# arielgabizon/barretenberg

Hardware: AMD Instinct MI355X
Metric: BN254 G1 MSM points/sec at n=2^20 (Fr NTT elems/sec in 'ntt') (higher is better)
Workload: dtype u32x9 (256-bit Montgomery, 29-bit limbs)

## Files before the change

### barretenberg_amd/csrc/msm.hip

```cpp
#include <hip/hip_runtime.h>

#include <algorithm>
#include <mutex>
#include <stdint.h>
#include <stdio.h>
#include <stdlib.h>
#include <string.h>
#include <vector>

#include "bbgpu_internal.h"
#include "g1.hpp"
#include "g1_quad.hpp"
#include "host_g1.hpp"

namespace bbgpu {

using Fr = FrP;
#ifndef BBGPU_FRONT_PRIO
#define BBGPU_FRONT_PRIO 2
#endif
#define FRONT_PRIO() __builtin_amdgcn_s_setprio(BBGPU_FRONT_PRIO)
#ifndef BBGPU_TAIL_PRIO
#define BBGPU_TAIL_PRIO 3
#endif
constexpr int SCALAR_BITS = 254;
constexpr int MSM_MAX_C = 16;
constexpr int MSM_THREADS = 256;

__device__ __forceinline__ void ld8(const uint32_t* p, uint32_t (&w)[8])
{
    const uint4* q = reinterpret_cast<const uint4*>(p);
    uint4 a = q[0], b = q[1];
    w[0] = a.x; w[1] = a.y; w[2] = a.z; w[3] = a.w;
    w[4] = b.x; w[5] = b.y; w[6] = b.z; w[7] = b.w;
}
__device__ __forceinline__ void ld16(const uint32_t* p, uint32_t (&w)[16])
{
    const uint4* q = reinterpret_cast<const uint4*>(p);
#pragma unroll
    for (int i = 0; i < 4; i++) {
        uint4 a = q[i];
        w[4 * i] = a.x; w[4 * i + 1] = a.y; w[4 * i + 2] = a.z; w[4 * i + 3] = a.w;
    }
}
__device__ __forceinline__ void st32(uint32_t* p, const uint32_t (&w)[32])
{
    uint4* q = reinterpret_cast<uint4*>(p);
#pragma unroll
    for (int i = 0; i < 8; i++) q[i] = make_uint4(w[4 * i], w[4 * i + 1], w[4 * i + 2], w[4 * i + 3]);
}
__device__ __forceinline__ void ld32(const uint32_t* p, uint32_t (&w)[32])
{
    const uint4* q = reinterpret_cast<const uint4*>(p);
#pragma unroll
    for (int i = 0; i < 8; i++) {
        uint4 a = q[i];
        w[4 * i] = a.x; w[4 * i + 1] = a.y; w[4 * i + 2] = a.z; w[4 * i + 3] = a.w;
    }
}

struct WinLayout {
    uint16_t off[66];
};
static WinLayout make_layout(int c, bool balanced)
{
    WinLayout LO{};
    const int W = msm_num_windows(c);
    if (!balanced) {
        for (int w = 0; w <= W; w++) LO.off[w] = (uint16_t)(c * w);
        return LO;
    }
    const int base = SCALAR_BITS / W, rem = SCALAR_BITS - base * W;
    int bit = 0;
    for (int w = 0; w < W; w++) {
        LO.off[w] = (uint16_t)bit;
        bit += base + (w < rem ? 1 : 0);
    }
    LO.off[W] = (uint16_t)bit;
    return LO;
}
__global__ void srs_convert_kernel(const uint32_t* __restrict__ table, uint32_t* __restrict__ srs, uint32_t n, uint32_t stride_words)
{
    const uint32_t i = blockIdx.x * blockDim.x + threadIdx.x;
    if (i >= n) return;
    uint32_t w[16];
    ld16(table + (size_t)i * stride_words, w);
    AffineV<2> a;
    load_affine_m256(a, w);
    uint32_t o[16];
    store_affine_m261(o, a.x, a.y);
    uint4* q = reinterpret_cast<uint4*>(srs + (size_t)i * 16);
#pragma unroll
    for (int k = 0; k < 4; k++) q[k] = make_uint4(o[4 * k], o[4 * k + 1], o[4 * k + 2], o[4 * k + 3]);
}

__global__ void srs_export_kernel(const uint32_t* __restrict__ srs, uint32_t* __restrict__ table, uint32_t n)
{
    const uint32_t i = blockIdx.x * blockDim.x + threadIdx.x;
    if (i >= n) return;
    uint32_t w[16];
    ld16(srs + (size_t)i * 16, w);
    AffineV<1> a;
    load_affine_m261(a, w);
    uint32_t o[8];
    uint32_t* dst = table + (size_t)i * 32;
    to_canonical(m261_to_m256<Fq>(a.x), o);
    for (int k = 0; k < 8; k++) dst[k] = o[k];
    to_canonical(m261_to_m256<Fq>(a.y), o);
    for (int k = 0; k < 8; k++) dst[8 + k] = o[k];
    auto bx = mul(a.x, fe_from<Fq>(Fq::BETA));
    to_canonical(m261_to_m256<Fq>(bx), o);
    for (int k = 0; k < 8; k++) dst[16 + k] = o[k];
    to_canonical(m261_to_m256<Fq>(weak(neg(a.y))), o);
    for (int k = 0; k < 8; k++) dst[24 + k] = o[k];
}


__global__ void __launch_bounds__(MSM_THREADS) srs_table_kernel(const uint32_t* __restrict__ srs, uint32_t* __restrict__ tab, uint32_t n, WinLayout LO,
                                                              uint32_t num_windows, uint32_t w_begin, uint32_t w_end)
{
    const uint32_t i = blockIdx.x * blockDim.x + threadIdx.x;
    if (i >= n) return;
    uint32_t w16[16];
    ld16(srs + (size_t)i * 16, w16);
    if (w_begin == 0) {
        uint4* q = reinterpret_cast<uint4*>(tab + (size_t)i * 16);
#pragma unroll
        for (int t = 0; t < 4; t++) q[t] = make_uint4(w16[4 * t], w16[4 * t + 1], w16[4 * t + 2], w16[4 * t + 3]);
    }
    AffineV<1> p;
    load_affine_m261(p, w16);
    Xyzz acc;
    from_affine(acc, p);
    for (uint32_t w = 1; w < num_windows && w < w_end; w++) {
        for (uint32_t k = LO.off[w - 1]; k < LO.off[w]; k++) {
            Xyzz t;
            dbl(t, acc);
            acc = t;
        }
        if (w < w_begin) continue;
        const uint64_t e[4] = { Fq::P64[0] - 2, Fq::P64[1], Fq::P64[2], Fq::P64[3] };
        auto inv = pow_u256<Fq>(mul(acc.zz, acc.zzz), e);
        auto izz = mul(inv, acc.zzz), izzz = mul(inv, acc.zz);
        uint32_t o[16];
        store_affine_m261(o, mul(acc.x, izz), mul(acc.y, izzz));
        uint4* q = reinterpret_cast<uint4*>(tab + ((size_t)w * n + i) * 16);
#pragma unroll
        for (int t = 0; t < 4; t++) q[t] = make_uint4(o[4 * t], o[4 * t + 1], o[4 * t + 2], o[4 * t + 3]);
    }
}

__global__ void srs_gen_table_kernel(uint32_t* __restrict__ tab)
{
    const uint32_t w = blockIdx.x * blockDim.x + threadIdx.x;
    if (w >= 32) return;
    Xyzz base;
    AffineV<1> g;
    g.x = fe_from<Fq>(Fq::GEN_X);
    g.y = fe_from<Fq>(Fq::GEN_Y);
    from_affine(base, g);
    for (uint32_t k = 0; k < 8 * w; k++) {
        Xyzz t;
        dbl(t, base);
        base = t;
    }
    Xyzz acc;
    set_infinity(acc);
    for (uint32_t d = 0; d < 256; d++) {
        uint32_t o[32];
        store_xyzz(o, acc);
        st32(tab + ((size_t)w * 256 + d) * 32, o);
        Xyzz t;
        add(t, acc, base);
        acc = t;
    }
}
__device__ __forceinline__ Fe<Fq, 1, 2> fq_inverse(const Fe<Fq, 1, 2>& a)
{
    const uint64_t e[4] = { Fq::P64[0] - 2, Fq::P64[1], Fq::P64[2], Fq::P64[3] };
    return pow_u256<Fq>(a, e);
}
__global__ void srs_gen_points_kernel(const uint32_t* __restrict__ tab, Limbs9 x261, uint32_t* __restrict__ srs, uint32_t n, uint32_t first)
{
    const uint32_t i = blockIdx.x * blockDim.x + threadIdx.x;
    if (i >= n) return;
    Fe<Fr, 1, 2> s = fe_one<Fr>(), b = fe_from<Fr>(x261.d);
    for (uint32_t e = first + i; e; e >>= 1) {
        if (e & 1) s = mul(s, b);
        b = sqr(b);
    }
    uint32_t k[8];
    {
        FeT<Fr> one_raw = fe_zero<Fr>();
        one_raw.d[0] = 1;
        to_canonical(mul(s, one_raw), k);
    }
    Xyzz acc;
    set_infinity(acc);
    for (uint32_t w = 0; w < 32; w++) {
        const uint32_t d = (k[w >> 2] >> ((w & 3) * 8)) & 0xff;
        if (d) {
            uint32_t pw[32];
            ld32(tab + ((size_t)w * 256 + d) * 32, pw);
            Xyzz q;
            load_xyzz(q, pw);
            Xyzz t;
            add(t, acc, q);
            acc = t;
        }
    }
    auto inv = fq_inverse(mul(acc.zz, acc.zzz));
    auto izz = mul(inv, acc.zzz), izzz = mul(inv, acc.zz);
    uint32_t o[16];
    store_affine_m261(o, mul(acc.x, izz), mul(acc.y, izzz));
    uint4* q = reinterpret_cast<uint4*>(srs + (size_t)i * 16);
#pragma unroll
    for (int t = 0; t < 4; t++) q[t] = make_uint4(o[4 * t], o[4 * t + 1], o[4 * t + 2], o[4 * t + 3]);
}

struct ScalarSets {
    const uint32_t* p[MSM_MAX_JOBS];
};
template <class DT> struct DigitTraits { static constexpr bool wide = false; };
template <> struct DigitTraits<uint16_t> { static constexpr bool wide = true; };
template <class DT> __device__ __forceinline__ int load_digit(const DT* __restrict__ dg, const unsigned long long* __restrict__ sg, uint32_t i)
{
    if constexpr (DigitTraits<DT>::wide) {
        const int u = dg[i];
        return ((sg[i >> 6] >> (i & 63u)) & 1ull) ? -u - 1 : u;
    } else {
        return dg[i];
    }
}
template <class DT> __device__ __forceinline__ void load_digits8(const DT* __restrict__ dg, const unsigned long long* __restrict__ sg, uint32_t i8, int (&d)[8])
{
    const uint4 q = *reinterpret_cast<const uint4*>(dg + i8);
    const uint32_t w[4] = { q.x, q.y, q.z, q.w };
    if constexpr (DigitTraits<DT>::wide) {
        const uint32_t sb = reinterpret_cast<const uint8_t*>(sg)[i8 >> 3];
#pragma unroll
        for (int k = 0; k < 8; k++) {
            const int u = (int)((w[k >> 1] >> (16 * (k & 1))) & 0xffffu);
            d[k] = ((sb >> k) & 1u) ? -u - 1 : u;
        }
    } else {
#pragma unroll
        for (int k = 0; k < 8; k++) d[k] = (int)(int16_t)(w[k >> 1] >> (16 * (k & 1)));
    }
}
template <class DT> __global__ void __launch_bounds__(MSM_THREADS) msm_digits_kernel(ScalarSets sets, DT* __restrict__ digits_all, unsigned long long* __restrict__ signs_all,
                                                               uint32_t n, WinLayout LO, uint32_t num_windows, uint32_t wb, uint32_t we)
{
    FRONT_PRIO();
    const uint32_t i = blockIdx.x * blockDim.x + threadIdx.x;
    if (i >= n) return;
    const uint32_t* __restrict__ scalars = sets.p[blockIdx.y];
    DT* __restrict__ digits = digits_all + (size_t)blockIdx.y * num_windows * n;
    const uint32_t s64 = (n + 63) >> 6;
    unsigned long long* __restrict__ signs = signs_all + (size_t)blockIdx.y * num_windows * s64;
    uint32_t w[8], k[9];
    ld8(scalars + (size_t)i * 8, w);
    to_canonical(exact_limbs(mul(unpack<Fr>(w), fe_from<Fr>(Fr::M256_TO_PLAIN))), w);
#pragma unroll
    for (int j = 0; j < 8; j++) k[j] = w[j];
    k[8] = 0;
    uint32_t carry = 0;
    for (uint32_t win = 0; win < we; win++) {
        const uint32_t bit = LO.off[win], sz = LO.off[win + 1] - bit, j = bit >> 5, s = bit & 31;
        const uint32_t half = 1u << (sz - 1), mask = (1u << sz) - 1;
        uint32_t v = 0;
        if (j < 8) {
            v = k[j] >> s;
            if (s + sz > 32) v |= k[j + 1] << (32 - s);
        }
        v = (v & mask) + carry;
        carry = (win + 1 < num_windows && v >= half) ? 1u : 0u;
        const int32_t d = (int32_t)v - (int32_t)(carry << sz);
        if (win >= wb) {
            if constexpr (DigitTraits<DT>::wide) {
                const unsigned long long neg = __ballot(d < 0);
                digits[(size_t)win * n + i] = (DT)(d < 0 ? -d - 1 : d);
                if ((threadIdx.x & 63u) == 0) signs[(size_t)win * s64 + (i >> 6)] = neg;
            } else {
                digits[(size_t)win * n + i] = (DT)d;
            }
        }
    }
}

constexpr int SORT_THREADS = 1024;
constexpr uint32_t SORT_MAX_LB = 7;
constexpr uint32_t SORTB_MAX_PARTS = 8;
constexpr uint32_t SORTB_SPLIT_MIN = 1u << 16;

__device__ __forceinline__ bool wave_keys_heavy(bool valid, uint32_t key)
{
    const uint64_t vm = __ballot(valid);
    if (!vm) return false;
    const uint32_t k0 = __builtin_amdgcn_readlane(key, __ffsll((unsigned long long)vm) - 1);
    return 4 * __popcll(__ballot(valid && key == k0)) >= __popcll(vm);
}
__device__ __forceinline__ uint32_t lds_inc_dedup(uint32_t* ctr, uint32_t key, bool heavy)
{
    if (!heavy) return atomicAdd(&ctr[key], 1u);
    const uint32_t lane = __lane_id();
    uint64_t todo = __ballot(1);
    uint32_t res = 0;
    for (int it = 0; it < 4 && todo; it++) {
        const int leader = __ffsll((unsigned long long)todo) - 1;
        const uint32_t kk = __builtin_amdgcn_readlane(key, leader);
        const uint64_t m = __ballot(key == kk) & todo;
        uint32_t base = 0;
        if ((int)lane == leader) base = atomicAdd(&ctr[kk], (uint32_t)__popcll(m));
        base = __builtin_amdgcn_readlane(base, leader);
        if ((m >> lane) & 1ull) res = base + (uint32_t)__popcll(m & ((1ull << lane) - 1ull));
        todo &= ~m;
    }
    if ((todo >> lane) & 1ull) res = atomicAdd(&ctr[key], 1u);
    return res;
}

template <class DT> __global__ void __launch_bounds__(SORT_THREADS) __attribute__((amdgpu_num_vgpr(32))) sortA_hist_kernel(const DT* __restrict__ digits, const unsigned long long* __restrict__ signs, uint32_t* __restrict__ histA, uint32_t n,
                                                                uint32_t bins, uint32_t lb, uint32_t slices, uint32_t slice_len, uint32_t win0,
                                                                uint32_t wpg, uint32_t first_i0, uint32_t last_i1, uint32_t blo, uint32_t bcnt)
{
    FRONT_PRIO();
    __shared__ uint32_t lh[SORT_THREADS];
    const uint32_t s = blockIdx.x, wl = blockIdx.y;
    lh[threadIdx.x] = 0;
    __syncthreads();
    const uint32_t lo = s * slice_len, hi = min(n, lo + slice_len);
    const uint32_t s64 = (n + 63) >> 6;
    if ((n & 7u) == 0) {
        const uint32_t lo8 = lo & ~7u, bpw = lo < hi ? (((hi + 7u) & ~7u) - lo8) >> 3 : 0u;
        for (uint32_t u = threadIdx.x; u < wpg * bpw; u += SORT_THREADS) {
            const uint32_t k = u / bpw, i8 = lo8 + (u - k * bpw) * 8;
            const uint32_t klo = (k == 0) ? max(lo, first_i0) : lo, khi = (k + 1 == wpg) ? min(hi, last_i1) : hi;
            int d[8];
            load_digits8<DT>(digits + (size_t)(win0 + wl * wpg + k) * n, signs + (size_t)(win0 + wl * wpg + k) * s64, i8, d);
            const bool heavy = wave_keys_heavy(d[0] != 0, (uint32_t)((d[0] < 0 ? -d[0] : d[0]) - 1) >> lb);
#pragma unroll
            for (int j = 0; j < 8; j++)
                if (d[j] && i8 + j >= klo && i8 + j < khi) {
                    const uint32_t b = (uint32_t)((d[j] < 0 ? -d[j] : d[j]) - 1);
                    if (b - blo < bcnt) (void)lds_inc_dedup(lh, b >> lb, heavy);
                }
        }
    } else {
        for (uint32_t k = 0; k < wpg; k++) {
            const DT* dg = digits + (size_t)(win0 + wl * wpg + k) * n;
            const unsigned long long* sg = signs + (size_t)(win0 + wl * wpg + k) * s64;
            const uint32_t klo = (k == 0) ? max(lo, first_i0) : lo, khi = (k + 1 == wpg) ? min(hi, last_i1) : hi;
            for (uint32_t i = klo + threadIdx.x; i < khi; i += SORT_THREADS) {
                const int d = load_digit<DT>(dg, sg, i);
                if (d) {
                    const uint32_t b = (uint32_t)((d < 0 ? -d : d) - 1);
                    if (b - blo < bcnt) atomicAdd(&lh[b >> lb], 1u);
                }
            }
        }
    }
    __syncthreads();
    if (threadIdx.x < bins) histA[((size_t)wl * slices + s) * bins + threadIdx.x] = lh[threadIdx.x];
}

__global__ void __launch_bounds__(SORT_THREADS) sortA_colscan_kernel(uint32_t* __restrict__ histA, uint32_t* __restrict__ bintot, uint32_t bins,
                                                                   uint32_t slices)
{
    FRONT_PRIO();
    const uint32_t wl = blockIdx.y, lane = threadIdx.x & 63;
    const uint32_t bin = blockIdx.x * (SORT_THREADS / 64) + (threadIdx.x >> 6);
    if (bin >= bins) return;
    uint32_t* H = histA + (size_t)wl * slices * bins + bin;
    const uint32_t spp = (slices + 63) / 64;
    const uint32_t s0 = min(slices, lane * spp), s1 = min(slices, s0 + spp);
    uint32_t sum = 0;
    for (uint32_t s = s0; s < s1; s++) sum += H[(size_t)s * bins];
    uint32_t incl = sum;
#pragma unroll
    for (int off = 1; off < 64; off <<= 1) {
        const uint32_t v = __shfl_up(incl, off);
        if ((int)lane >= off) incl += v;
    }
    uint32_t run = incl - sum;
    for (uint32_t s = s0; s < s1; s++) {
        const uint32_t cnt = H[(size_t)s * bins];
        H[(size_t)s * bins] = run;
        run += cnt;
    }
    if (lane == 63) bintot[(size_t)wl * bins + bin] = incl;
}
__global__ void __launch_bounds__(SORT_THREADS) sortA_scan_kernel(const uint32_t* __restrict__ bintot, uint32_t* __restrict__ binstart,
                                                                uint32_t* __restrict__ totals, uint32_t bins, uint32_t* __restrict__ solo_bases,
                                                                uint32_t* __restrict__ solo_gstart_end)
{
    FRONT_PRIO();
    __shared__ uint32_t part[SORT_THREADS];
    const uint32_t wl = blockIdx.x, t = threadIdx.x;
    const uint32_t mine = t < bins ? bintot[(size_t)wl * bins + t] : 0;
    part[t] = mine;
    __syncthreads();
    for (uint32_t off = 1; off < SORT_THREADS; off <<= 1) {
        uint32_t v = t >= off ? part[t - off] : 0;
        __syncthreads();
        part[t] += v;
        __syncthreads();
    }
    if (t < bins) binstart[(size_t)wl * bins + t] = part[t] - mine;
    if (t == SORT_THREADS - 1) {
        totals[wl] = part[SORT_THREADS - 1];
        if (solo_bases) {
            solo_bases[0] = 0;
            solo_bases[1] = part[SORT_THREADS - 1];
            solo_gstart_end[0] = part[SORT_THREADS - 1];
            solo_gstart_end[1] = 0xffffffffu;
        }
    }
}
__global__ void sort_bases_kernel(const uint32_t* __restrict__ totals, uint32_t* __restrict__ bases, uint32_t* __restrict__ gstart_end, uint32_t nw)
{
    FRONT_PRIO();
    if (threadIdx.x == 0 && blockIdx.x == 0) {
        uint32_t run = 0;
        for (uint32_t w = 0; w < nw; w++) {
            bases[w] = run;
            run += totals[w];
        }
        bases[nw] = run;
        gstart_end[0] = run;
        gstart_end[1] = 0xffffffffu;
    }
}


template <class DT> __global__ void __launch_bounds__(SORT_THREADS) __attribute__((amdgpu_num_vgpr(32))) sortA_scatter_kernel(const DT* __restrict__ digits, const unsigned long long* __restrict__ signs, const uint32_t* __restrict__ cursorsA,
                                                                   const uint32_t* __restrict__ binstart, const uint32_t* __restrict__ bases,
                                                                   uint32_t* __restrict__ tmp, uint32_t n, uint32_t bins, uint32_t lb,
                                                                   uint32_t slices, uint32_t slice_len, uint32_t win0, uint32_t wpg,
                                                                   uint32_t idx_stride, uint32_t windows_per_job, uint32_t first_i0, uint32_t last_i1, uint32_t blo, uint32_t bcnt)
{
    FRONT_PRIO();
    __shared__ uint32_t lc[SORT_THREADS];
    const uint32_t s = blockIdx.x, wl = blockIdx.y;
    if (threadIdx.x < bins)
        lc[threadIdx.x] = cursorsA[((size_t)wl * slices + s) * bins + threadIdx.x] + binstart[(size_t)wl * bins + threadIdx.x] + bases[wl];
    __syncthreads();
    const uint32_t lo = s * slice_len, hi = min(n, lo + slice_len);
    const uint32_t lomask = (1u << lb) - 1;
    const uint32_t s64 = (n + 63) >> 6;
    if ((n & 7u) == 0) {
        const uint32_t lo8 = lo & ~7u, bpw = lo < hi ? (((hi + 7u) & ~7u) - lo8) >> 3 : 0u;
        for (uint32_t u = threadIdx.x; u < wpg * bpw; u += SORT_THREADS) {
            const uint32_t k = u / bpw, i8 = lo8 + (u - k * bpw) * 8;
            const uint32_t wabs = win0 + wl * wpg + k;
            const uint32_t row = (wabs % windows_per_job) * idx_stride;
            const uint32_t klo = (k == 0) ? max(lo, first_i0) : lo, khi = (k + 1 == wpg) ? min(hi, last_i1) : hi;
            int d[8];
            load_digits8<DT>(digits + (size_t)wabs * n, signs + (size_t)wabs * s64, i8, d);
#pragma unroll
            for (int j = 0; j < 8; j++) {
                if (d[j] && i8 + j >= klo && i8 + j < khi) {
                    const uint32_t b = (uint32_t)((d[j] < 0 ? -d[j] : d[j]) - 1);
                    if (b - blo < bcnt) {
                        const uint32_t pos = atomicAdd(&lc[b >> lb], 1u);
                        tmp[pos] = (row + i8 + j) | ((b & lomask) << 24) | (d[j] < 0 ? 0x80000000u : 0u);
                    }
                }
            }
        }
        return;
    }
    for (uint32_t k = 0; k < wpg; k++) {
        const uint32_t wabs = win0 + wl * wpg + k;
        const DT* dg = digits + (size_t)wabs * n;
        const unsigned long long* sg = signs + (size_t)wabs * s64;
        const uint32_t row = (wabs % windows_per_job) * idx_stride;
        const uint32_t klo = (k == 0) ? max(lo, first_i0) : lo, khi = (k + 1 == wpg) ? min(hi, last_i1) : hi;
        for (uint32_t i = klo + threadIdx.x; i < khi; i += SORT_THREADS) {
            const int d = load_digit<DT>(dg, sg, i);
            if (d) {
                const uint32_t b = (uint32_t)((d < 0 ? -d : d) - 1);
                if (b - blo < bcnt) {
                    const uint32_t pos = atomicAdd(&lc[b >> lb], 1u);
                    tmp[pos] = (row + i) | ((b & lomask) << 24) | (d < 0 ? 0x80000000u : 0u);
                }
            }
        }
    }
}

template <class DT> __global__ void __launch_bounds__(SORT_THREADS) __attribute__((amdgpu_waves_per_eu(8, 8))) sortA_scatter_staged_kernel(const DT* __restrict__ digits, const unsigned long long* __restrict__ signs, const uint32_t* __restrict__ cursorsA,
                                                                          const uint32_t* __restrict__ binstart, const uint32_t* __restrict__ bases,
                                                                          uint32_t* __restrict__ tmp, uint32_t n, uint32_t bins, uint32_t lb,
                                                                          uint32_t slices, uint32_t slice_len, uint32_t win0, uint32_t wpg,
                                                                          uint32_t idx_stride, uint32_t windows_per_job, uint32_t first_i0, uint32_t last_i1, uint32_t blo, uint32_t bcnt)
{
    FRONT_PRIO();
    constexpr uint32_t TILE = SORT_THREADS * 8;
    __shared__ uint32_t lc[SORT_THREADS];
    __shared__ uint32_t th[SORT_THREADS];
    __shared__ uint32_t dlt[SORT_THREADS];
    __shared__ uint32_t wsum[SORT_THREADS / 64 + 1];
    __shared__ uint32_t buf[TILE];
    __shared__ uint16_t bbin[TILE];
    const uint32_t s = blockIdx.x, wl = blockIdx.y, t = threadIdx.x, lane = t & 63, wave = t >> 6;
    lc[t] = t < bins ? cursorsA[((size_t)wl * slices + s) * bins + t] + binstart[(size_t)wl * bins + t] + bases[wl] : 0u;
    const uint32_t lo = s * slice_len, hi = min(n, lo + slice_len);
    const uint32_t lomask = (1u << lb) - 1;
    const uint32_t s64 = (n + 63) >> 6;
    const uint32_t lo8 = lo & ~7u, bpw = lo < hi ? (((hi + 7u) & ~7u) - lo8) >> 3 : 0u;
    const uint32_t total_u = wpg * bpw;
    for (uint32_t u0 = 0; u0 < total_u; u0 += SORT_THREADS) {
        th[t] = 0;
        __syncthreads();
        uint32_t ent[8], bn[8], rk[8];
        const uint32_t u = u0 + t;
#pragma unroll
        for (int j = 0; j < 8; j++) bn[j] = 0xffffffffu;
        if (u < total_u) {
            const uint32_t k = u / bpw, i8 = lo8 + (u - k * bpw) * 8;
            const uint32_t wabs = win0 + wl * wpg + k;
            const uint32_t row = (wabs % windows_per_job) * idx_stride;
            const uint32_t klo = (k == 0) ? max(lo, first_i0) : lo, khi = (k + 1 == wpg) ? min(hi, last_i1) : hi;
            int d[8];
            load_digits8<DT>(digits + (size_t)wabs * n, signs + (size_t)wabs * s64, i8, d);
            const bool heavy = wave_keys_heavy(d[0] != 0, (uint32_t)((d[0] < 0 ? -d[0] : d[0]) - 1) >> lb);
#pragma unroll
            for (int j = 0; j < 8; j++) {
                if (d[j] && i8 + j >= klo && i8 + j < khi) {
                    const uint32_t b = (uint32_t)((d[j] < 0 ? -d[j] : d[j]) - 1);
                    if (b - blo < bcnt) {
                        bn[j] = b >> lb;
                        ent[j] = (row + i8 + j) | ((b & lomask) << 24) | (d[j] < 0 ? 0x80000000u : 0u);
                        rk[j] = lds_inc_dedup(th, bn[j], heavy);
                    }
                }
            }
        }
        __syncthreads();
        const uint32_t c = th[t];
        uint32_t incl = c;
#pragma unroll
        for (int off = 1; off < 64; off <<= 1) {
            const uint32_t o = __shfl_up(incl, off);
            if ((int)lane >= off) incl += o;
        }
        if (lane == 63) wsum[wave] = incl;
        __syncthreads();
        uint32_t before = 0;
        for (uint32_t w = 0; w < wave; w++) before += wsum[w];
        const uint32_t excl = before + incl - c;
        th[t] = excl;
        const uint32_t g = lc[t];
        dlt[t] = g - excl;
        lc[t] = g + c;
        if (t == SORT_THREADS - 1) wsum[SORT_THREADS / 64] = excl + c;
        __syncthreads();
#pragma unroll
        for (int j = 0; j < 8; j++) {
            if (bn[j] != 0xffffffffu) {
                const uint32_t slot = th[bn[j]] + rk[j];
                buf[slot] = ent[j];
                bbin[slot] = (uint16_t)bn[j];
            }
        }
        __syncthreads();
        const uint32_t tile_n = wsum[SORT_THREADS / 64];
        for (uint32_t x = t; x < tile_n; x += SORT_THREADS) tmp[dlt[bbin[x]] + x] = buf[x];
    }
}

__global__ void __launch_bounds__(SORT_THREADS) sortB_kernel(const uint32_t* __restrict__ tmp, const uint32_t* __restrict__ binstart,
                                                   const uint32_t* __restrict__ bases, uint32_t* __restrict__ sorted, uint32_t* __restrict__ gstart,
                                                   uint32_t bins, uint32_t lb, uint32_t nb)
{
    FRONT_PRIO();
    __shared__ uint32_t cnt[128];
    __shared__ uint32_t cur[128];
    const uint32_t bin = blockIdx.x, wl = blockIdx.y, t = threadIdx.x;
    const uint32_t nlo = 1u << lb;
    const uint32_t start = bases[wl] + binstart[(size_t)wl * bins + bin];
    const uint32_t end = (bin + 1 < bins) ? bases[wl] + binstart[(size_t)wl * bins + bin + 1] : bases[wl + 1];
    if (t < 128) cnt[t] = 0;
    __syncthreads();
    constexpr int UB = 8;
    for (uint32_t e0 = start + t; e0 < end; e0 += UB * blockDim.x) {
        uint32_t v[UB];
#pragma unroll
        for (int k = 0; k < UB; k++) {
            const uint32_t e = e0 + k * blockDim.x;
            v[k] = e < end ? tmp[e] : 0u;
        }
#pragma unroll
        for (int k = 0; k < UB; k++)
            if (e0 + k * blockDim.x < end) atomicAdd(&cnt[(v[k] >> 24) & 0x7f], 1u);
    }
    __syncthreads();
    if (t < 64) {
        const uint32_t a = cnt[2 * t], b2 = cnt[2 * t + 1], sum = a + b2;
        uint32_t incl = sum;
#pragma unroll
        for (int off = 1; off < 64; off <<= 1) {
            const uint32_t o = __shfl_up(incl, off);
            if ((int)t >= off) incl += o;
        }
        cur[2 * t] = start + incl - sum;
        cur[2 * t + 1] = start + incl - sum + a;
    }
    __syncthreads();
    if (t < nlo) gstart[(size_t)wl * nb + (size_t)bin * nlo + t] = cur[t];
    __syncthreads();
    for (uint32_t e0 = start + t; e0 < end; e0 += UB * blockDim.x) {
        uint32_t v[UB];
#pragma unroll
        for (int k = 0; k < UB; k++) {
            const uint32_t e = e0 + k * blockDim.x;
            v[k] = e < end ? tmp[e] : 0u;
        }
#pragma unroll
        for (int k = 0; k < UB; k++) {
            if (e0 + k * blockDim.x < end) {
                const uint32_t pos = atomicAdd(&cur[(v[k] >> 24) & 0x7f], 1u);
                sorted[pos] = v[k] & 0x80ffffffu;
            }
        }
    }
}

template <int THREADS> __global__ void __launch_bounds__(THREADS) sortB_count_kernel(const uint32_t* __restrict__ tmp, const uint32_t* __restrict__ binstart,
                                                                                       const uint32_t* __restrict__ bases, uint32_t* __restrict__ histB, uint32_t bins, uint32_t parts)
{
    FRONT_PRIO();
    constexpr int UB = 8;
    constexpr uint32_t TILE = THREADS * UB;
    __shared__ uint32_t cnt[128];
    const uint32_t bin = blockIdx.x, wl = blockIdx.y, part = blockIdx.z, t = threadIdx.x;
    const uint32_t bstart = bases[wl] + binstart[(size_t)wl * bins + bin];
    const uint32_t bend = (bin + 1 < bins) ? bases[wl] + binstart[(size_t)wl * bins + bin + 1] : bases[wl + 1];
    const uint32_t len = bend - bstart;
    if (len <= SORTB_SPLIT_MIN) return;
    const uint32_t start = bstart + (uint32_t)(((uint64_t)len * part) / parts), end = bstart + (uint32_t)(((uint64_t)len * (part + 1)) / parts);
    if (t < 128) cnt[t] = 0;
    __syncthreads();
    for (uint32_t e0 = start + t; e0 < end; e0 += TILE) {
        uint32_t v[UB];
#pragma unroll
        for (int k = 0; k < UB; k++) {
            const uint32_t e = e0 + k * THREADS;
            v[k] = e < end ? tmp[e] : 0u;
        }
        const bool heavy = wave_keys_heavy(e0 < end, (v[0] >> 24) & 0x7f);
#pragma unroll
        for (int k = 0; k < UB; k++)
            if (e0 + k * THREADS < end) (void)lds_inc_dedup(cnt, (v[k] >> 24) & 0x7f, heavy);
    }
    __syncthreads();
    if (t < 128) histB[(((size_t)wl * bins + bin) * parts + part) * 128 + t] = cnt[t];
}
template <int THREADS> __global__ void __launch_bounds__(THREADS) sortB_staged_kernel(const uint32_t* __restrict__ tmp, const uint32_t* __restrict__ binstart,
                                                                                        const uint32_t* __restrict__ bases, uint32_t* __restrict__ sorted,
                                                                                        uint32_t* __restrict__ gstart, uint32_t bins, uint32_t lb, uint32_t nb,
                                                                                        const uint32_t* __restrict__ histB, uint32_t parts_launched)
{
    FRONT_PRIO();
    constexpr int UB = 8;
    constexpr uint32_t TILE = THREADS * UB;
    __shared__ uint32_t cnt[128];
    __shared__ uint32_t cur[128];
    __shared__ uint32_t toff[128];
    __shared__ uint32_t dlt[128];
    __shared__ uint32_t bef[128];
    __shared__ uint32_t buf[TILE];
    const uint32_t bin = blockIdx.x, wl = blockIdx.y, part = blockIdx.z, t = threadIdx.x;
    const uint32_t nlo = 1u << lb;
    const uint32_t bstart = bases[wl] + binstart[(size_t)wl * bins + bin];
    const uint32_t bend = (bin + 1 < bins) ? bases[wl] + binstart[(size_t)wl * bins + bin + 1] : bases[wl + 1];
    const uint32_t len = bend - bstart;
    const uint32_t parts = (parts_launched > 1 && len > SORTB_SPLIT_MIN) ? parts_launched : 1u;
    if (part >= parts) return;
    const uint32_t start = bstart + (uint32_t)(((uint64_t)len * part) / parts), end = bstart + (uint32_t)(((uint64_t)len * (part + 1)) / parts);
    if (t < 128) {
        uint32_t total = 0, before = 0;
        if (parts > 1) {
            const uint32_t* h = histB + (((size_t)wl * bins + bin) * parts) * 128 + t;
            for (uint32_t p = 0; p < parts; p++) {
                const uint32_t c = h[(size_t)p * 128];
                total += c;
                if (p < part) before += c;
            }
        }
        cnt[t] = total;
        bef[t] = before;
    }
    __syncthreads();
    for (uint32_t e0 = start + t; parts == 1 && e0 < end; e0 += TILE) {
        uint32_t v[UB];
#pragma unroll
        for (int k = 0; k < UB; k++) {
            const uint32_t e = e0 + k * THREADS;
            v[k] = e < end ? tmp[e] : 0u;
        }
        const bool heavy = wave_keys_heavy(e0 < end, (v[0] >> 24) & 0x7f);
#pragma unroll
        for (int k = 0; k < UB; k++)
            if (e0 + k * THREADS < end) (void)lds_inc_dedup(cnt, (v[k] >> 24) & 0x7f, heavy);
    }
    __syncthreads();
    if (t < 64) {
        const uint32_t a = cnt[2 * t], b2 = cnt[2 * t + 1], sum = a + b2;
        uint32_t incl = sum;
#pragma unroll
        for (int off = 1; off < 64; off <<= 1) {
            const uint32_t o = __shfl_up(incl, off);
            if ((int)t >= off) incl += o;
        }
        cur[2 * t] = bstart + incl - sum;
        cur[2 * t + 1] = bstart + incl - sum + a;
    }
    __syncthreads();
    if (t < nlo && part == 0) gstart[(size_t)wl * nb + (size_t)bin * nlo + t] = cur[t];
    __syncthreads();
    if (t < 128) cur[t] += bef[t];
    __syncthreads();
    for (uint32_t base = start; base < end; base += TILE) {
        if (t < 128) cnt[t] = 0;
        __syncthreads();
        uint32_t v[UB], rk[UB];
#pragma unroll
        for (int k = 0; k < UB; k++) {
            const uint32_t e = base + k * THREADS + t;
            v[k] = e < end ? tmp[e] : 0u;
        }
        const bool heavy = wave_keys_heavy(base + t < end, (v[0] >> 24) & 0x7f);
#pragma unroll
        for (int k = 0; k < UB; k++) {
            rk[k] = 0u;
            if (base + k * THREADS + t < end) rk[k] = lds_inc_dedup(cnt, (v[k] >> 24) & 0x7f, heavy);
        }
        __syncthreads();
        if (t < 64) {
            const uint32_t a = cnt[2 * t], b2 = cnt[2 * t + 1], sum = a + b2;
            uint32_t incl = sum;
#pragma unroll
            for (int off = 1; off < 64; off <<= 1) {
                const uint32_t o = __shfl_up(incl, off);
                if ((int)t >= off) incl += o;
            }
            const uint32_t x0 = incl - sum, x1 = x0 + a;
            toff[2 * t] = x0;
            toff[2 * t + 1] = x1;
            const uint32_t c0 = cur[2 * t], c1 = cur[2 * t + 1];
            dlt[2 * t] = c0 - x0;
            dlt[2 * t + 1] = c1 - x1;
            cur[2 * t] = c0 + a;
            cur[2 * t + 1] = c1 + b2;
        }
        __syncthreads();
#pragma unroll
        for (int k = 0; k < UB; k++)
            if (base + k * THREADS + t < end) buf[toff[(v[k] >> 24) & 0x7f] + rk[k]] = v[k];
        __syncthreads();
        const uint32_t tile_n = min(TILE, end - base);
        for (uint32_t x = t; x < tile_n; x += THREADS) {
            const uint32_t w = buf[x];
            sorted[dlt[(w >> 24) & 0x7f] + x] = w & 0x80ffffffu;
        }
    }
}

__device__ __forceinline__ void store_raw(uint32_t* dst, const Xyzz& p)
{
#if defined(__HIP_DEVICE_COMPILE__) && !defined(BBGPU_STORE_RAW_X4)
    uint32_t v[4 * NL];
#pragma unroll
    for (int i = 0; i < NL; i++) { v[i] = p.x.d[i]; v[NL + i] = p.y.d[i]; v[2 * NL + i] = p.zz.d[i]; v[3 * NL + i] = p.zzz.d[i]; }
#pragma unroll
    for (int i = 0; i < 4 * NL; i += 2)
        asm volatile("global_store_dwordx2 %0, %1, off offset:%2" :: "v"(dst), "v"(((unsigned long long)v[i + 1] << 32) | v[i]), "n"(4 * i) : "memory");
#else
#pragma unroll
    for (int i = 0; i < NL; i++) {
        dst[i] = p.x.d[i];
        dst[NL + i] = p.y.d[i];
        dst[2 * NL + i] = p.zz.d[i];
        dst[3 * NL + i] = p.zzz.d[i];
    }
#endif
}
__device__ __forceinline__ void load_raw(Xyzz& p, const uint32_t* src)
{
#pragma unroll
    for (int i = 0; i < NL; i++) {
        p.x.d[i] = src[i];
        p.y.d[i] = src[NL + i];
        p.zz.d[i] = src[2 * NL + i];
        p.zzz.d[i] = src[3 * NL + i];
    }
}
#ifdef BBGPU_ACC_CAP128
#define ACC_VGPR_CAP __attribute__((amdgpu_waves_per_eu(4, 4)))
#else
#define ACC_VGPR_CAP
#endif
constexpr int RAW_WORDS = 4 * NL;
constexpr uint32_t HEAVY_WGS = 256;
constexpr uint32_t HEAVY_IDS = 1 + HEAVY_WGS;
static_assert(MSM_THREADS == (int)HEAVY_WGS, "heavy-bucket queue header is cleared / combined by one lane per K4h workgroup");

__global__ void __launch_bounds__(MSM_THREADS) ACC_VGPR_CAP msm_accumulate_kernel(const uint32_t* __restrict__ srs, const uint32_t* __restrict__ sorted,
                                                                   const uint32_t* __restrict__ gstart, uint32_t* __restrict__ partials,
                                                                   uint32_t total_buckets, uint32_t ch, uint32_t prio, uint32_t* __restrict__ heavy_counter)
{
    if (heavy_counter && blockIdx.x == 0) {
        heavy_counter[threadIdx.x] = 0;
        if (threadIdx.x == 0) heavy_counter[MSM_THREADS] = 0;
    }
    if (prio == 1) __builtin_amdgcn_s_setprio(1);
    else if (prio == 2) __builtin_amdgcn_s_setprio(2);
    const uint32_t t = blockIdx.x * blockDim.x + threadIdx.x;
    const uint32_t M = gstart[total_buckets];
    const uint32_t p0 = t * ch;
    if (p0 >= M) return;
    const uint32_t p1 = min(M, p0 + ch);
    uint32_t lo = 0, hi = total_buckets;
    while (hi - lo > 1) {
        const uint32_t mid = (lo + hi) >> 1;
        if (gstart[mid] <= p0) lo = mid; else hi = mid;
    }
    uint32_t b = lo;
    uint32_t next_end = gstart[b + 1];
    Xyzz acc;
    set_infinity(acc);
    uint32_t after_next = gstart[min(b + 2, total_buckets + 1)];
    bool acc_inf = true;
    uint32_t v = sorted[p0];
    uint32_t vn = sorted[p0 + 1 < p1 ? p0 + 1 : p0];
    uint32_t w[16];
    ld16(srs + (size_t)(v & 0x7fffffffu) * 16, w);
    Fe<Fq, 1, 1> px;
    Fe<Fq, 1, 2> py;
    load_affine_m261_signed(px, py, w, (v >> 31) != 0);
    ld16(srs + (size_t)(vn & 0x7fffffffu) * 16, w);
    uint32_t e = p0;
    uint32_t trips = ch;
    do {
        const uint32_t vnn = sorted[min(e + 2, p1 - 1)];
        const bool start = (e == next_end) || acc_inf;
        if (start) {
            if (e == next_end) {
                store_raw(partials + (size_t)(b + t) * RAW_WORDS, acc);
                b++;
                next_end = after_next;
                if (next_end <= e) {
                    if (e >= M) {
                        b = total_buckets;
                    } else {
                        uint32_t l2 = b, h2 = total_buckets;
                        while (h2 - l2 > 1) {
                            const uint32_t mid = (l2 + h2) >> 1;
                            if (gstart[mid] <= e) l2 = mid; else h2 = mid;
                        }
                        b = l2;
                    }
                    next_end = gstart[b + 1];
                }
                after_next = gstart[min(b + 2, total_buckets + 1)];
            }
            acc.x = px;
            acc.y = py;
            acc.zz = fe_one<Fq>();
            acc.zzz = fe_one<Fq>();
            acc_inf = false;
        }
        asm volatile("" ::: "memory");
        if (!start) madd_ip(acc, acc_inf, px, py);
#ifdef BBGPU_ACC_JUNK
        {
            uint32_t j0 = e, j1 = vn;
#pragma unroll
            for (int q = 0; q < BBGPU_ACC_JUNK / 2; q++) asm volatile("v_and_b32 %0, 0x1fffffff, %1\n\tv_add_u32 %1, %0, %1" : "+v"(j0), "+v"(j1));
        }
#endif
#ifdef BBGPU_ACC_JUNKMAD
        {
            unsigned long long ja = e;
#pragma unroll
            for (int q = 0; q < BBGPU_ACC_JUNKMAD; q++) asm volatile("v_mad_u64_u32 %0, vcc, %1, %1, %0" : "+v"(ja) : "v"(vn) : "vcc");
        }
#endif
        load_affine_m261_signed(px, py, w, (vn >> 31) != 0);
        ld16(srs + (size_t)(vnn & 0x7fffffffu) * 16, w);
        vn = vnn;
        e++;
    } while (--trips != 0);
    store_raw(partials + (size_t)(b + t) * RAW_WORDS, acc);
}

__device__ __forceinline__ Xyzz shfl_down_xyzz(const Xyzz& p, uint32_t off)
{
    Xyzz r;
#pragma unroll
    for (int i = 0; i < NL; i++) {
        r.x.d[i] = __shfl_down(p.x.d[i], off);
        r.y.d[i] = __shfl_down(p.y.d[i], off);
        r.zz.d[i] = __shfl_down(p.zz.d[i], off);
        r.zzz.d[i] = __shfl_down(p.zzz.d[i], off);
    }
    return r;
}
#ifndef BBGPU_TAIL_WAVES
#define BBGPU_TAIL_WAVES 4
#endif
#define TAIL_OCC __attribute__((amdgpu_waves_per_eu(BBGPU_TAIL_WAVES, BBGPU_TAIL_WAVES)))
constexpr int FOLD_T = 256;
constexpr int FOLD_LDS_WORDS = (FOLD_T / 2) * RAW_WORDS;
__device__ __forceinline__ void wg_tree_sum(Xyzz& acc, uint32_t* sh, uint32_t T, uint32_t t)
{
    constexpr uint32_t STRIDE = FOLD_T / 2;
    for (uint32_t half = T >> 1; half >= 1; half >>= 1) {
        if (t >= half && t < 2 * half) {
#pragma unroll
            for (int i = 0; i < NL; i++) {
                sh[(0 * NL + i) * STRIDE + t - half] = acc.x.d[i];
                sh[(1 * NL + i) * STRIDE + t - half] = acc.y.d[i];
                sh[(2 * NL + i) * STRIDE + t - half] = acc.zz.d[i];
                sh[(3 * NL + i) * STRIDE + t - half] = acc.zzz.d[i];
            }
        }
        __syncthreads();
        if (t < half) {
            Xyzz q, r;
#pragma unroll
            for (int i = 0; i < NL; i++) {
                q.x.d[i] = sh[(0 * NL + i) * STRIDE + t];
                q.y.d[i] = sh[(1 * NL + i) * STRIDE + t];
                q.zz.d[i] = sh[(2 * NL + i) * STRIDE + t];
                q.zzz.d[i] = sh[(3 * NL + i) * STRIDE + t];
            }
            add(r, acc, q);
            acc = r;
        }
        __syncthreads();
    }
}
__global__ void __launch_bounds__(MSM_THREADS) TAIL_OCC msm_merge_kernel(const uint32_t* __restrict__ gstart, const uint32_t* __restrict__ partials,
                                                              uint32_t* __restrict__ buckets, uint32_t* __restrict__ heavy, uint32_t bucket_begin, uint32_t total_buckets,
                                                              uint32_t ch, uint32_t MERGE_LIGHT, uint32_t logG)
{
    __builtin_amdgcn_s_setprio(BBGPU_TAIL_PRIO);
    const uint32_t t = blockIdx.x * blockDim.x + threadIdx.x;
    const uint32_t G = 1u << logG, b = bucket_begin + (t >> logG), j = t & (G - 1);
    if (b >= total_buckets) return;
    const uint32_t s = gstart[b], e = gstart[b + 1];
    Xyzz acc;
    set_infinity(acc);
    if (e > s) {
        const uint32_t t0 = s / ch, t1 = (e - 1) / ch;
        if (t1 - t0 >= MERGE_LIGHT) {
            if (j == 0) heavy[HEAVY_IDS + atomicAdd(&heavy[0], 1u)] = b;
            return;
        }
        for (uint32_t k = t0 + j; k <= t1; k += G) {
            Xyzz q, r;
            load_raw(q, partials + (size_t)(b + k) * RAW_WORDS);
            add(r, acc, q);
            acc = r;
        }
    }
    for (uint32_t off = G >> 1; off >= 1; off >>= 1) {
        const Xyzz o = shfl_down_xyzz(acc, off);
        if (j < off) {
            Xyzz r;
            add(r, acc, o);
            acc = r;
        }
    }
    if (j == 0) {
        uint32_t o[32];
        store_xyzz(o, acc);
        st32(buckets + (size_t)b * 32, o);
    }
}
__global__ void __launch_bounds__(MSM_THREADS) TAIL_OCC msm_merge_heavy_kernel(const uint32_t* __restrict__ gstart, const uint32_t* __restrict__ partials,
                                                                    uint32_t* __restrict__ buckets, uint32_t* __restrict__ heavy, uint32_t ch, uint32_t* __restrict__ hpart)
{
    __builtin_amdgcn_s_setprio(BBGPU_TAIL_PRIO);
    __shared__ uint32_t sh[FOLD_LDS_WORDS];
    __shared__ uint32_t last_flag;
    const uint32_t count = heavy[0];
    const uint32_t K = count ? gridDim.x / count : 0;
    if (K < 2) {
        for (uint32_t item = blockIdx.x; item < count; item += gridDim.x) {
            const uint32_t b = heavy[HEAVY_IDS + item];
            const uint32_t s = gstart[b], e = gstart[b + 1];
            const uint32_t t0 = s / ch, t1 = (e - 1) / ch;
            Xyzz acc;
            set_infinity(acc);
            for (uint32_t t = t0 + threadIdx.x; t <= t1; t += MSM_THREADS) {
                Xyzz q, r;
                load_raw(q, partials + (size_t)(b + t) * RAW_WORDS);
                add(r, acc, q);
                acc = r;
            }
            __syncthreads();
            wg_tree_sum(acc, sh, MSM_THREADS, threadIdx.x);
            if (threadIdx.x == 0) {
                uint32_t o[32];
                store_xyzz(o, acc);
                st32(buckets + (size_t)b * 32, o);
            }
        }
        return;
    }
    const uint32_t item = blockIdx.x / K, sub = blockIdx.x - item * K;
    if (item >= count) return;
    const uint32_t b = heavy[HEAVY_IDS + item];
    const uint32_t s = gstart[b], e = gstart[b + 1];
    const uint32_t t0 = s / ch, t1 = (e - 1) / ch, total = t1 - t0 + 1;
    const uint32_t lo = t0 + (uint32_t)(((uint64_t)total * sub) / K), hi = t0 + (uint32_t)(((uint64_t)total * (sub + 1)) / K);
    Xyzz acc;
    set_infinity(acc);
    for (uint32_t t = lo + threadIdx.x; t < hi; t += MSM_THREADS) {
        Xyzz q, r;
        load_raw(q, partials + (size_t)(b + t) * RAW_WORDS);
        add(r, acc, q);
        acc = r;
    }
    wg_tree_sum(acc, sh, MSM_THREADS, threadIdx.x);
    if (threadIdx.x == 0) {
        store_raw(hpart + (size_t)blockIdx.x * RAW_WORDS, acc);
        __threadfence();
        last_flag = (atomicAdd(&heavy[1 + item], 1u) == K - 1) ? 1u : 0u;
    }
    __syncthreads();
    if (!last_flag) return;
    __threadfence();
    set_infinity(acc);
    if (threadIdx.x < K) load_raw(acc, hpart + (size_t)(item * K + threadIdx.x) * RAW_WORDS);
    __syncthreads();
    wg_tree_sum(acc, sh, MSM_THREADS, threadIdx.x);
    if (threadIdx.x == 0) {
        uint32_t o[32];
        store_xyzz(o, acc);
        st32(buckets + (size_t)b * 32, o);
    }
}

__device__ __forceinline__ uint32_t insert_one_bit(uint32_t m, uint32_t k)
{
    return ((m >> k) << (k + 1)) | (1u << k) | (m & ((1u << k) - 1));
}

__global__ void __launch_bounds__(FOLD_T) TAIL_OCC msm_rowcol_kernel(const uint32_t* __restrict__ buckets, uint32_t* __restrict__ R, uint32_t* __restrict__ Cc,
                                                          uint32_t H, uint32_t L, uint32_t* __restrict__ zero_out, uint32_t zero_words)
{
    __builtin_amdgcn_s_setprio(BBGPU_TAIL_PRIO);
    __shared__ uint32_t sh[FOLD_LDS_WORDS];
    const uint32_t g = blockIdx.y, t = threadIdx.x, nb = H * L;
    if (zero_out) {
        const uint32_t gid = (g * gridDim.x + blockIdx.x) * blockDim.x + t, all = gridDim.y * gridDim.x * blockDim.x;
        for (uint32_t i = gid; i < zero_words; i += all) zero_out[i] = 0;
    }
    const bool row = blockIdx.x < H;
    const uint32_t idx = row ? blockIdx.x : blockIdx.x - H, count = row ? L : H;
    Xyzz acc;
    set_infinity(acc);
    if (t < count) {
        const size_t b = row ? (size_t)idx * L + t : (size_t)t * L + idx;
        uint32_t w[32];
        ld32(buckets + ((size_t)g * nb + b) * 32, w);
        load_xyzz(acc, w);
    }
    wg_tree_sum(acc, sh, blockDim.x, t);
    if (t == 0) {
        uint32_t w[32];
        store_xyzz(w, acc);
        st32((row ? R + ((size_t)g * H + idx) * 32 : Cc + ((size_t)g * L + idx) * 32), w);
    }
}
__global__ void __launch_bounds__(FOLD_T) TAIL_OCC msm_final_kernel(const uint32_t* __restrict__ R, const uint32_t* __restrict__ Cc, uint32_t* __restrict__ out,
                                                         uint32_t hbits, uint32_t lbits)
{
    __builtin_amdgcn_s_setprio(BBGPU_TAIL_PRIO);
    __shared__ uint32_t sh[FOLD_LDS_WORDS];
    const uint32_t g = blockIdx.y, t = threadIdx.x, job = blockIdx.x;
    const uint32_t H = 1u << hbits, L = 1u << lbits;
    const uint32_t* src;
    uint32_t count, slot, k = 0;
    bool sliced = true;
    if (job == 0) { src = R + (size_t)g * H * 32; count = H; slot = 0; sliced = false; }
    else if (job < 1 + hbits) { k = job - 1; src = R + (size_t)g * H * 32; count = H >> 1; slot = 1 + k; }
    else { k = job - 1 - hbits; src = Cc + (size_t)g * L * 32; count = L >> 1; slot = 32 + k; }
    Xyzz acc;
    set_infinity(acc);
    if (t < count) {
        uint32_t w[32];
        ld32(src + (size_t)(sliced ? insert_one_bit(t, k) : t) * 32, w);
        load_xyzz(acc, w);
    }
    wg_tree_sum(acc, sh, blockDim.x, t);
    if (t == 0) {
        uint32_t o[32];
        store_xyzz_m256(o, acc);
        st32(out + ((size_t)g * 64 + slot) * 32, o);
    }
}

constexpr int QFOLD_T = 256;
__device__ __forceinline__ FqN quad_load(const uint32_t* point32, uint32_t l)
{
    const uint4* q = reinterpret_cast<const uint4*>(point32 + 8 * l);
    const uint4 a = q[0], b = q[1];
    const uint32_t w[8] = { a.x, a.y, a.z, a.w, b.x, b.y, b.z, b.w };
    return FqN(unpack<Fq>(w));
}
__device__ __forceinline__ FqN quad_zero()
{
    return FqN(fe_zero<Fq>());
}
template <int T = QFOLD_T> __device__ __forceinline__ FqN block_quad_sum(FqN acc, uint32_t* sh , uint32_t t, uint32_t active = T / 4)
{
    const uint32_t l = t & 3, lane = t & 63, wave = t >> 6, qd = lane >> 2;
    const uint32_t in_wave = active > 16 * wave ? min(16u, active - 16 * wave) : 0u;
    for (uint32_t off = 8; off >= 1; off >>= 1) {
        if (off >= in_wave) continue;
        FqN o;
#pragma unroll
        for (int i = 0; i < NL; i++) o.d[i] = __shfl_down(acc.d[i], off * 4);
        if (qd < off) acc = quad_add(acc, o, l);
    }
    if constexpr (T == 64) return acc;
    constexpr uint32_t NW = T / 64;
    const uint32_t waves = min(NW, (active + 15) / 16);
    if (waves <= 1) return acc;
    if (lane < 4) {
#pragma unroll
        for (int i = 0; i < NL; i++) sh[(wave * 4 + l) * NL + i] = acc.d[i];
    }
    __syncthreads();
    if (wave == 0) {
        acc = quad_zero();
        if (qd < NW) {
#pragma unroll
            for (int i = 0; i < NL; i++) acc.d[i] = sh[(qd * 4 + l) * NL + i];
        }
        for (uint32_t off = NW >> 1; off >= 1; off >>= 1) {
            if (off >= waves) continue;
            FqN o;
#pragma unroll
            for (int i = 0; i < NL; i++) o.d[i] = __shfl_down(acc.d[i], off * 4);
            if (qd < off) acc = quad_add(acc, o, l);
        }
    }
    return acc;
}
__device__ __forceinline__ void quad_store8(uint32_t* dst8, const uint32_t (&w)[8])
{
    uint4* q = reinterpret_cast<uint4*>(dst8);
    q[0] = make_uint4(w[0], w[1], w[2], w[3]);
    q[1] = make_uint4(w[4], w[5], w[6], w[7]);
}

__global__ void __launch_bounds__(MSM_THREADS) TAIL_OCC msm_merge_quad_kernel(const uint32_t* __restrict__ gstart, const uint32_t* __restrict__ partials,
                                                                   uint32_t* __restrict__ buckets, uint32_t* __restrict__ heavy, uint32_t bucket_begin, uint32_t total_buckets,
                                                                   uint32_t ch, uint32_t MERGE_LIGHT, uint32_t logQ)
{
    __builtin_amdgcn_s_setprio(BBGPU_TAIL_PRIO);
    const uint32_t t = blockIdx.x * blockDim.x + threadIdx.x, l = t & 3, quad = t >> 2;
    const uint32_t Q = 1u << logQ, b = bucket_begin + (quad >> logQ), j = quad & (Q - 1);
    if (b >= total_buckets) return;
    const uint32_t s = gstart[b], e = gstart[b + 1];
    FqN acc = quad_zero();
    if (e > s) {
        const uint32_t t0 = s / ch, t1 = (e - 1) / ch;
        if (t1 - t0 >= MERGE_LIGHT) {
            if (j == 0 && l == 0) heavy[HEAVY_IDS + atomicAdd(&heavy[0], 1u)] = b;
            return;
        }
        uint32_t k = t0 + j;
        if (k <= t1) {
            const uint32_t* src = partials + (size_t)(b + k) * RAW_WORDS + NL * l;
#pragma unroll
            for (int i = 0; i < NL; i++) acc.d[i] = src[i];
            FqN q = quad_zero();
            k += Q;
            if (k <= t1) {
                src = partials + (size_t)(b + k) * RAW_WORDS + NL * l;
#pragma unroll
                for (int i = 0; i < NL; i++) q.d[i] = src[i];
            }
            while (k <= t1) {
                FqN qn = quad_zero();
                const uint32_t kn = k + Q;
                if (kn <= t1) {
                    src = partials + (size_t)(b + kn) * RAW_WORDS + NL * l;
#pragma unroll
                    for (int i = 0; i < NL; i++) qn.d[i] = src[i];
                }
                acc = quad_add(acc, q, l);
                q = qn;
                k = kn;
            }
        }
    }
    for (uint32_t off = Q >> 1; off >= 1; off >>= 1) {
        FqN o;
#pragma unroll
        for (int i = 0; i < NL; i++) o.d[i] = __shfl_down(acc.d[i], off * 4);
        if (j < off) acc = quad_add(acc, o, l);
    }
    if (j == 0) {
        uint32_t w[8];
        to_canonical(acc, w);
        quad_store8(buckets + (size_t)b * 32 + 8 * l, w);
    }
}

__global__ void __launch_bounds__(QFOLD_T) TAIL_OCC msm_rowcol_quad_kernel(const uint32_t* __restrict__ buckets, uint32_t* __restrict__ R, uint32_t* __restrict__ Cc,
                                                                  uint32_t H, uint32_t L, uint32_t* __restrict__ zero_out, uint32_t zero_words, uint32_t r0, uint32_t rows)
{
    __builtin_amdgcn_s_setprio(BBGPU_TAIL_PRIO);
    __shared__ uint32_t sh[(QFOLD_T / 64) * 4 * NL];
    const uint32_t g = blockIdx.y, t = threadIdx.x, nb = H * L, l = t & 3, quad = t >> 2;
    if (zero_out) {
        const uint32_t gid = (g * gridDim.x + blockIdx.x) * blockDim.x + t, all = gridDim.y * gridDim.x * blockDim.x;
        for (uint32_t i = gid; i < zero_words; i += all) zero_out[i] = 0;
    }
    const bool row = blockIdx.x < rows;
    const uint32_t idx = row ? r0 + blockIdx.x : blockIdx.x - rows, count = row ? L : rows;
    FqN acc = quad_zero();
    bool first = true;
    for (uint32_t e = quad; e < count; e += QFOLD_T / 4) {
        const size_t b = row ? (size_t)idx * L + e : (size_t)(r0 + e) * L + idx;
        const FqN v = quad_load(buckets + ((size_t)g * nb + b) * 32, l);
        acc = first ? v : quad_add(acc, v, l);
        first = false;
    }
    acc = block_quad_sum(acc, sh, t, min(count, (uint32_t)QFOLD_T / 4));
    if (t < 4) {
        uint32_t w[8];
        to_canonical(acc, w);
        quad_store8((row ? R + ((size_t)g * H + idx) * 32 : Cc + ((size_t)g * L + idx) * 32) + 8 * l, w);
    }
}
constexpr uint32_t ROWCOL_SEG = 4;
__global__ void __launch_bounds__(MSM_THREADS) TAIL_OCC msm_rowcol_seg_kernel(const uint32_t* __restrict__ buckets, uint32_t* __restrict__ segs, uint32_t H, uint32_t L,
                                                                                                                uint32_t* __restrict__ zero_out, uint32_t zero_words)
{
    __builtin_amdgcn_s_setprio(BBGPU_TAIL_PRIO);
    const uint32_t g = blockIdx.y, t = blockIdx.x * blockDim.x + threadIdx.x, nb = H * L;
    if (zero_out) {
        const uint32_t gid = g * gridDim.x * blockDim.x + t, all = gridDim.y * gridDim.x * blockDim.x;
        for (uint32_t i = gid; i < zero_words; i += all) zero_out[i] = 0;
    }
    const uint32_t row_lanes = H * (L / ROWCOL_SEG), col_lanes = L * (H / ROWCOL_SEG);
    if (t >= row_lanes + col_lanes) return;
    size_t b, step, out;
    if (t < row_lanes) {
        const uint32_t per = L / ROWCOL_SEG, r = t / per, sidx = t - r * per;
        b = (size_t)r * L + sidx;
        step = per;
        out = t;
    } else {
        const uint32_t u = t - row_lanes, per = H / ROWCOL_SEG, sidx = u / L, c = u - sidx * L;
        b = (size_t)sidx * L + c;
        step = (size_t)per * L;
        out = (size_t)row_lanes + (size_t)c * per + sidx;
    }
    const uint32_t* src = buckets + ((size_t)g * nb + b) * 32;
    Xyzz acc;
    {
        uint32_t w[32];
        ld32(src, w);
        load_xyzz(acc, w);
    }
    for (uint32_t j = 1; j < ROWCOL_SEG; j++) {
        uint32_t w[32];
        ld32(src + j * step * 32, w);
        Xyzz q, r;
        load_xyzz(q, w);
        add(r, acc, q);
        acc = r;
    }
    uint32_t o[32];
    store_xyzz(o, acc);
    st32(segs + ((size_t)g * (row_lanes + col_lanes) + out) * 32, o);
}
__global__ void __launch_bounds__(64) TAIL_OCC msm_segsum_quad_kernel(const uint32_t* __restrict__ segs, uint32_t* __restrict__ R, uint32_t* __restrict__ Cc, uint32_t H, uint32_t L)
{
    __builtin_amdgcn_s_setprio(BBGPU_TAIL_PRIO);
    const uint32_t g = blockIdx.y, t = threadIdx.x, l = t & 3, quad = t >> 2;
    const uint32_t row_lanes = H * (L / ROWCOL_SEG), col_lanes = L * (H / ROWCOL_SEG);
    const bool row = blockIdx.x < H;
    const uint32_t idx = row ? blockIdx.x : blockIdx.x - H, count = row ? L / ROWCOL_SEG : H / ROWCOL_SEG;
    const uint32_t* src = segs + ((size_t)g * (row_lanes + col_lanes) + (row ? (size_t)idx * count : (size_t)row_lanes + (size_t)idx * count)) * 32;
    FqN acc = quad_zero();
    bool first = true;
    for (uint32_t e = quad; e < count; e += 16) {
        const FqN v = quad_load(src + (size_t)e * 32, l);
        acc = first ? v : quad_add(acc, v, l);
        first = false;
    }
    acc = block_quad_sum<64>(acc, nullptr, t, min(count, 16u));
    if (t < 4) {
        uint32_t w[8];
        to_canonical(acc, w);
        quad_store8((row ? R + ((size_t)g * H + idx) * 32 : Cc + ((size_t)g * L + idx) * 32) + 8 * l, w);
    }
}
__global__ void __launch_bounds__(QFOLD_T) TAIL_OCC msm_final_quad_kernel(const uint32_t* __restrict__ R, const uint32_t* __restrict__ Cc, uint32_t* __restrict__ out,
                                                                 uint32_t hbits, uint32_t lbits)
{
    __builtin_amdgcn_s_setprio(BBGPU_TAIL_PRIO);
    __shared__ uint32_t sh[(QFOLD_T / 64) * 4 * NL];
    const uint32_t g = blockIdx.y, t = threadIdx.x, job = blockIdx.x, l = t & 3, quad = t >> 2;
    const uint32_t H = 1u << hbits, L = 1u << lbits;
    const uint32_t* src;
    uint32_t count, slot, k = 0;
    bool sliced = true;
    if (job == 0) { src = R + (size_t)g * H * 32; count = H; slot = 0; sliced = false; }
    else if (job < 1 + hbits) { k = job - 1; src = R + (size_t)g * H * 32; count = H >> 1; slot = 1 + k; }
    else { k = job - 1 - hbits; src = Cc + (size_t)g * L * 32; count = L >> 1; slot = 32 + k; }
    FqN acc = quad_zero();
    bool first = true;
    for (uint32_t e = quad; e < count; e += QFOLD_T / 4) {
        const FqN v = quad_load(src + (size_t)(sliced ? insert_one_bit(e, k) : e) * 32, l);
        acc = first ? v : quad_add(acc, v, l);
        first = false;
    }
    acc = block_quad_sum(acc, sh, t, min(count, (uint32_t)QFOLD_T / 4));
    if (t < 4) {
        uint32_t w[8];
        to_canonical(m261_to_m256<Fq>(acc), w);
        quad_store8(out + ((size_t)g * 64 + slot) * 32 + 8 * l, w);
    }
}

#define HIPCHK(x)                                                                                                      \
    do {                                                                                                               \
        hipError_t e_ = (x);                                                                                           \
        if (e_ != hipSuccess) {                                                                                        \
            set_error("%s:%d %s -> %s", __FILE__, __LINE__, #x, hipGetErrorString(e_));                                \
            return BBGPU_ERR_HIP;                                                                                      \
        }                                                                                                              \
    } while (0)

int msm_choose_c(size_t n)
{
    int lg = 0;
    while (((size_t)1 << lg) < n) lg++;
    int c = lg - 4;
    if (c < 4) c = 4;
    if (c > MSM_MAX_C) c = MSM_MAX_C;
    return c;
}
int msm_num_windows(int c)
{
    return SCALAR_BITS / c + 1;
}

struct MsmPlan {
    uint32_t n, c, W, nb, hbits, lbits, slices, slice_len, sort_lb, sort_bins;
};
constexpr uint32_t ACC_LDS_RESERVE = 41 * 1024;
static uint32_t acc_wg_per_cu()
{
    static int v = 0;
    if (!v) {
        v = 3;
        if (const char* e = getenv("BBGPU_ACC_WGS")) v = std::min(4, std::max(1, atoi(e)));
    }
    return (uint32_t)v;
}
static uint32_t acc_lds_reserve()
{
    static int v = -1;
    if (v < 0) {
        v = acc_wg_per_cu() == 3 ? (int)ACC_LDS_RESERVE : (acc_wg_per_cu() == 2 ? 60 * 1024 : 0);
        if (const char* e = getenv("BBGPU_ACC_LDS")) v = std::min(64 * 1024, std::max(0, atoi(e)));
    }
    return (uint32_t)v;
}
static uint32_t acc_prio()
{
    static int v = -1;
    if (v < 0) {
        v = 0;
        if (const char* e = getenv("BBGPU_ACC_PRIO")) v = std::min(2, std::max(0, atoi(e)));
    }
    return (uint32_t)v;
}
static uint32_t acc_capacity_lanes()
{
    static uint32_t lanes = 0;
    if (!lanes) {
        int dev = 0, cus = 256;
        (void)hipGetDevice(&dev);
        (void)hipDeviceGetAttribute(&cus, hipDeviceAttributeMultiprocessorCount, dev);
        lanes = (uint32_t)cus * acc_wg_per_cu() * MSM_THREADS;
    }
    return lanes;
}
constexpr uint32_t MIN_CHUNK = 8;
constexpr uint64_t TINY_ENTRIES = (uint64_t)1 << 16;
constexpr uint32_t TINY_MIN_CHUNK = 4;
static uint32_t min_chunk(uint64_t m) { return m <= TINY_ENTRIES ? TINY_MIN_CHUNK : MIN_CHUNK; }
static uint32_t chunk_len_m(uint64_t m);
static bool chunk_forced()
{
    static const bool f = getenv("BBGPU_CHUNK") != nullptr || getenv("BBGPU_ACC_WAVES") != nullptr;
    return f;
}
static uint32_t chunk_len(size_t n, uint32_t nw)
{
    return chunk_len_m((uint64_t)n * nw);
}
static uint32_t chunk_len_m(const uint64_t m)
{
    static int waves = 0;
    if (!waves) {
        waves = 1;
        if (const char* e = getenv("BBGPU_ACC_WAVES")) waves = std::min(16, std::max(1, atoi(e)));
    }
    static const int forced = [] { const char* e = getenv("BBGPU_CHUNK"); return e ? std::max((int)MIN_CHUNK, atoi(e)) : 0; }();
    if (forced) return (uint32_t)std::max<uint64_t>(forced, (m + ((uint64_t)1 << 24) - 1) >> 24);
    if (waves > 1) {
        const uint64_t cap = (uint64_t)acc_capacity_lanes() * (uint64_t)waves;
        return std::max<uint32_t>(MIN_CHUNK, (uint32_t)((m + cap - 1) / cap));
    }
    static const double step[3] = { 6.4, 9.2, 13.4 };
    const uint64_t per_k = (uint64_t)acc_capacity_lanes() / acc_wg_per_cu();
    uint32_t best = 0;
    double best_cost = 0.0;
    for (uint32_t k = 1; k <= acc_wg_per_cu() && k <= 3; k++) {
        const uint32_t ch = std::max<uint32_t>(min_chunk(m), (uint32_t)((m + per_k * k - 1) / (per_k * k)));
        const double cost = ch * step[k - 1];
        if (!best || cost < best_cost) { best = ch; best_cost = cost; }
    }
    return best;
}
static size_t arena_points(const MsmPlan& P, uint32_t nw)
{
    const size_t H = (size_t)1 << P.hbits, L = (size_t)1 << P.lbits;
    return (size_t)nw * (H + L) + 64;
}
static bool rowcol_two_step(const MsmPlan& P)
{
    return P.hbits + P.lbits >= 15;
}
static size_t seg_points(const MsmPlan& P, uint32_t nw)
{
    const size_t H = (size_t)1 << P.hbits, L = (size_t)1 << P.lbits;
    return rowcol_two_step(P) ? (size_t)nw * 2 * (H * L / ROWCOL_SEG) : 0;
}
static MsmPlan make_plan(size_t n, int c)
{
    MsmPlan P;
    P.n = (uint32_t)n;
    P.c = (uint32_t)c;
    P.W = (uint32_t)msm_num_windows(c);
    P.nb = 1u << (c - 1);
    P.lbits = (c - 1) / 2;
    P.hbits = (c - 1) - P.lbits;
    P.slices = std::max<uint32_t>(1, 512 / P.W);
    P.sort_lb = std::min<uint32_t>(SORT_MAX_LB, (uint32_t)c - 1);
    P.sort_bins = P.nb >> P.sort_lb;
    if ((uint64_t)P.slices * 4096 > n) P.slices = std::max<uint32_t>(1, (uint32_t)(n / 4096));
    P.slice_len = (uint32_t)((n + P.slices - 1) / P.slices);
    return P;
}

struct MsmCarve {
    size_t digits, signs, histA, histB, binstart, bintot, tmp_entries, gstart, totals, heavy, sorted, partials, buckets, arena, segs, texp, end;
    size_t chunks_cap, histB_bytes;
};
static MsmCarve carve(const MsmPlan& P, size_t n, size_t nw, size_t ng)
{
    auto al = [](size_t x) { return (x + 255) & ~(size_t)255; };
    MsmCarve L;
    size_t p = 0;
    const size_t wmax = std::max<size_t>(P.W, nw);
    L.digits = p;      p += al(wmax * n * 2);
    L.signs = p;       p += al(wmax * ((n + 63) / 64) * 8);
    L.histA = p;       p += al(nw * P.slices * 1024 * 4);
    L.histB_bytes = (uint64_t)n * nw >= ((uint64_t)1 << 21) ? (size_t)MSM_MAX_JOBS * 1024 * SORTB_MAX_PARTS * 128 * 4 : 0;
    L.histB = p;       p += al(L.histB_bytes);
    L.binstart = p;    p += al(nw * 1024 * 4 + 256);
    L.bintot = p;      p += al(nw * 1024 * 4 + 256);
    L.tmp_entries = p; p += al(nw * n * 4);
    L.gstart = p;      p += al((ng * P.nb + 2) * 4);
    L.totals = p;      p += al(nw * 8 + 512);
    L.heavy = p;       p += al((ng * P.nb + HEAVY_IDS) * 4 + 256 + (size_t)HEAVY_WGS * RAW_WORDS * 4);
    L.sorted = p;      p += al(nw * n * 4);
    L.chunks_cap = (n * nw + min_chunk(n * nw) - 1) / min_chunk(n * nw) + 1;
    L.partials = p;    p += al((ng * P.nb + L.chunks_cap) * RAW_WORDS * 4);
    L.buckets = p;     p += al(ng * P.nb * 128);
    L.arena = p;       p += al(arena_points(P, (uint32_t)ng) * 128);
    L.segs = p;        p += al(seg_points(P, (uint32_t)ng) * 128);
    L.texp = p;        p += al(ng * 64 * 128);
    L.end = p;
    return L;
}
size_t MsmWorkspace::bytes_needed(size_t n, int c, int nw, int ng)
{
    return carve(make_plan(n, c), n, (size_t)nw, (size_t)(ng > 0 ? ng : nw)).end;
}

int MsmWorkspace::ensure(size_t bytes)
{
    if (bytes <= cap) return BBGPU_OK;
    if (base) (void)dev_free(base);
    base = nullptr;
    cap = 0;
    HIPCHK(dev_malloc((void**)&base, bytes));
    cap = bytes;
    return BBGPU_OK;
}
void MsmWorkspace::release()
{
    if (base) (void)dev_free(base);
    if (h_out) (void)hipHostFree(h_out);
    base = nullptr;
    h_out = nullptr;
    cap = 0;
}

int msm_issue(MsmSlot& S, const uint32_t* d_srs, const uint32_t* d_tab, size_t tab_stride, int tab_c, const uint64_t* d_scalars, size_t n, int wb,
              int we, hipStream_t st, int want_timing)
{
    return msm_issue_batch(S, d_srs, d_tab, tab_stride, tab_c, &d_scalars, 1, n, wb, we, st, want_timing, 0, (uint32_t)n);
}
int msm_issue_rows(MsmSlot& S, const uint32_t* d_srs, const uint32_t* d_tab, size_t tab_stride, int tab_c, const uint64_t* d_scalars, size_t n,
                   uint64_t row_begin, uint64_t row_end, hipStream_t st, int want_timing)
{
    if (!d_tab || n == 0 || row_end <= row_begin || row_end > (uint64_t)msm_num_windows(tab_c) * n) return BBGPU_ERR_ARG;
    const int wb = (int)(row_begin / n), we = (int)((row_end + n - 1) / n);
    const uint32_t i0 = (uint32_t)(row_begin - (uint64_t)wb * n), i1 = (uint32_t)(row_end - (uint64_t)(we - 1) * n);
    return msm_issue_batch(S, d_srs, d_tab, tab_stride, tab_c, &d_scalars, 1, n, wb, we, st, want_timing, i0, i1);
}

int msm_issue_buckets(MsmSlot& S, const uint32_t* d_srs, const uint32_t* d_tab, size_t tab_stride, int tab_c, const uint64_t* d_scalars, size_t n,
                      uint32_t share, uint32_t share_count, hipStream_t st, int want_timing)
{
    if (!d_tab || n == 0 || share_count == 0 || share >= share_count) return BBGPU_ERR_ARG;
    const MsmPlan P = make_plan(n, tab_c);
    const uint32_t H = 1u << P.hbits;
    if (share_count > H) return BBGPU_ERR_ARG;
    const uint32_t r0 = (uint32_t)((uint64_t)H * share / share_count), r1 = (uint32_t)((uint64_t)H * (share + 1) / share_count);
    return msm_issue_batch(S, d_srs, d_tab, tab_stride, tab_c, &d_scalars, 1, n, 0, (int)P.W, st, want_timing, 0, 0xffffffffu, r0, r1);
}

constexpr int ACC_RING = 8;
static hipEvent_t g_acc_end[ACC_RING];
static uint64_t g_acc_seq = 0;
static int acc_ring_record(MsmSlot& S, hipStream_t st)
{
    if (g_acc_seq == 0)
        for (int i = 0; i < ACC_RING; i++) HIPCHK(hipEventCreate(&g_acc_end[i]));
    S.acc_seq = ++g_acc_seq;
    HIPCHK(hipEventRecord(g_acc_end[S.acc_seq % ACC_RING], st));
    return BBGPU_OK;
}
int msm_issue_batch(MsmSlot& S, const uint32_t* d_srs, const uint32_t* d_tab, size_t tab_stride, int tab_c, const uint64_t* const* d_scalars_v, int jobs,
                    size_t n, int wb, int we, hipStream_t st, int want_timing, uint32_t row_i0, uint32_t row_i1, uint32_t brow0, uint32_t brow1)
{
    MsmWorkspace& ws = S.ws;
    const bool append = S.append && S.pending && S.npieces > 0;
    S.append = false;
    if (append && (S.jobs != (uint32_t)jobs || S.npieces >= MSM_MAX_PIECES)) {
        set_error("internal: MSM piece %d does not continue the MSM on this slot", S.npieces);
        return BBGPU_ERR_STATE;
    }
    if (!append) {
        S.jobs = (uint32_t)jobs;
        S.n = n;
        S.pending = false;
        S.timed = false;
        S.npieces = 0;
    } else {
        S.n += n;
    }
    MsmPiece& PC = S.piece[S.npieces];
    PC = MsmPiece{};
    PC.hout_group = S.npieces ? S.piece[S.npieces - 1].hout_group + S.piece[S.npieces - 1].nw : 0u;
    if (n == 0) { PC.trivial = true; S.npieces++; S.pending = true; return BBGPU_OK; }
    if (n > ((size_t)1 << 24)) {
        set_error("MSM of %zu points: at most 2^24 points per call", n);
        return BBGPU_ERR_SIZE;
    }
    const bool hint = S.throughput;
    S.throughput = false;
    const bool table = d_tab != nullptr;
    const int c = table ? tab_c : msm_choose_c(n);
    const MsmPlan P = make_plan(n, c);
    if (wb < 0 || we > (int)P.W || wb >= we) return BBGPU_ERR_ARG;
    if (row_i1 > n) row_i1 = (uint32_t)n;
    if ((row_i0 != 0 || row_i1 != n) && (!table || jobs != 1 || row_i0 >= n || (we - wb == 1 && row_i0 >= row_i1))) return BBGPU_ERR_ARG;
    if (jobs < 1 || jobs > MSM_MAX_JOBS || (jobs > 1 && (!table || wb != 0 || we != (int)P.W))) {
        set_error("batched MSM: 1..%d jobs, window tables and the full window range required", MSM_MAX_JOBS);
        return BBGPU_ERR_ARG;
    }
    const uint32_t BH = 1u << P.hbits, BL = 1u << P.lbits;
    if (brow1 > BH) brow1 = BH;
    const bool bshare = brow0 != 0 || brow1 != BH;
    if (bshare && (!table || jobs != 1 || brow0 >= brow1 || wb != 0 || we != (int)P.W || row_i0 != 0 || row_i1 != n)) return BBGPU_ERR_ARG;
    const uint32_t blo = brow0 * BL, bcnt = (brow1 - brow0) * BL;
    const uint32_t nw1 = (uint32_t)(we - wb);
    const uint32_t nw = nw1 * (uint32_t)jobs;
    const uint32_t G = table ? (uint32_t)jobs : nw1;
    const uint32_t wpg = table ? nw1 : 1u;
    uint32_t sort_lb = P.sort_lb, sort_bins = P.sort_bins;
    if (table) {
        uint32_t want_bins = 512;
        if (const char* e = getenv("BBGPU_SORT_BINS")) want_bins = std::min(1024, std::max(64, atoi(e)));
        while (sort_bins < want_bins && sort_lb > 3) { sort_lb--; sort_bins <<= 1; }
    }
    uint32_t slices = table ? std::max<uint32_t>(1, P.slices * nw1 / 2) : P.slices;
    if (table && jobs == 1) {
        const uint32_t by_cap = (uint32_t)(((uint64_t)nw * P.slices * 1024) / ((uint64_t)G * sort_bins));
        const uint32_t want = std::min<uint32_t>(std::min<uint32_t>(208, (uint32_t)(n / 2048)), by_cap);
        slices = std::max(slices, want);
    }
    if (const char* e = getenv("BBGPU_SLICES")) slices = std::min<uint32_t>(std::max(1, atoi(e)), P.slices * nw1);
    const uint32_t slice_len = (uint32_t)((n + slices - 1) / slices);
    const uint32_t idx_stride = table ? (uint32_t)tab_stride : 0u;
    const uint32_t* points = table ? d_tab : d_srs;
    PC.c = P.c; PC.nw = G; PC.wb = table ? 0u : (uint32_t)wb; PC.hbits = P.hbits; PC.lbits = P.lbits;
    if (PC.hout_group + G > MSM_HOUT_GROUPS) {
        set_error("MSM in %d pieces of %u bucket sets: the result array holds %u", S.npieces + 1, G, MSM_HOUT_GROUPS);
        return BBGPU_ERR_SIZE;
    }
    int rc = ws.ensure(MsmWorkspace::bytes_needed(n, c, (int)nw, (int)G));
    if (rc) return rc;
    if (!ws.h_out) HIPCHK(hipHostMalloc((void**)&ws.h_out, (size_t)MSM_HOUT_GROUPS * 64 * 128));
    if (!S.done) HIPCHK(hipEventCreateWithFlags(&S.done, hipEventDisableTiming));

    const MsmCarve LY = carve(P, n, nw, G);
    if (LY.end > ws.cap) {
        set_error("internal: MSM workspace of %zu bytes, layout needs %zu (n=%zu c=%d nw=%u)", ws.cap, LY.end, n, c, nw);
        return BBGPU_ERR_STATE;
    }
    uint8_t* const p = ws.base;
    void* digits = (void*)(p + LY.digits);
    unsigned long long* signs = (unsigned long long*)(p + LY.signs);
    uint32_t* histA = (uint32_t*)(p + LY.histA);
    uint32_t* histB = (uint32_t*)(p + LY.histB);
    uint32_t* binstart = (uint32_t*)(p + LY.binstart);
    uint32_t* bintot = (uint32_t*)(p + LY.bintot);
    uint32_t* tmp_entries = (uint32_t*)(p + LY.tmp_entries);
    uint32_t* gstart = (uint32_t*)(p + LY.gstart);
    uint32_t* totals = (uint32_t*)(p + LY.totals);
    uint32_t* bases = totals + nw;
    uint32_t* heavy = (uint32_t*)(p + LY.heavy);
    uint32_t* sorted = (uint32_t*)(p + LY.sorted);
    uint32_t* partials = (uint32_t*)(p + LY.partials);
    uint32_t* buckets = (uint32_t*)(p + LY.buckets);
    uint32_t* scratch = (uint32_t*)(p + LY.arena);
    uint32_t* texp = (uint32_t*)(p + LY.texp);
    if ((uint64_t)G * slices * sort_bins > (uint64_t)nw * P.slices * 1024 || sort_bins > 1024 ||
        (size_t)G * ((size_t)(1u << P.hbits) + (size_t)(1u << P.lbits)) + 64 > arena_points(P, G)) {
        set_error("internal: MSM launch shape exceeds the workspace layout");
        return BBGPU_ERR_STATE;
    }

    hipEvent_t* ev = S.ev;
    const bool tm = want_timing == 1, tm_acc = want_timing != 0;
    S.timed_light = want_timing == 2;
    if (tm_acc) {
        if (!S.ev[0])
            for (int i = 0; i < 8; i++) HIPCHK(hipEventCreate(&S.ev[i]));
        if (tm) HIPCHK(hipEventRecord(ev[0], st));
        S.timed = true;
    }

    if (bshare) {
        static const bool quad_ok = [] { const char* e = getenv("BBGPU_QUAD_TAIL"); return !e || atoi(e) != 0; }();
        if (!quad_ok) {
            set_error("bucket-range shares need the quad tail kernels (BBGPU_QUAD_TAIL=0 is set)");
            return BBGPU_ERR_STATE;
        }
        HIPCHK(hipMemsetAsync(scratch, 0, (size_t)G * BH * 128, st));
    }
    ScalarSets sets{};
    for (int j = 0; j < jobs; j++) sets.p[j] = (const uint32_t*)d_scalars_v[j];
    const bool wide = c > 16;
    if (wide) msm_digits_kernel<uint16_t><<<dim3((P.n + MSM_THREADS - 1) / MSM_THREADS, jobs), MSM_THREADS, 0, st>>>(sets, (uint16_t*)digits, signs, P.n, make_layout(c, table), P.W, (uint32_t)wb, (uint32_t)we);
    else msm_digits_kernel<int16_t><<<dim3((P.n + MSM_THREADS - 1) / MSM_THREADS, jobs), MSM_THREADS, 0, st>>>(sets, (int16_t*)digits, signs, P.n, make_layout(c, table), P.W, (uint32_t)wb, (uint32_t)we);
    if (tm) HIPCHK(hipEventRecord(ev[1], st));
    if (wide) sortA_hist_kernel<uint16_t><<<dim3(slices, G), SORT_THREADS, 0, st>>>((const uint16_t*)digits, signs, histA, P.n, sort_bins, sort_lb, slices, slice_len, (uint32_t)wb, wpg, row_i0, row_i1, blo, bcnt);
    else sortA_hist_kernel<int16_t><<<dim3(slices, G), SORT_THREADS, 0, st>>>((const int16_t*)digits, signs, histA, P.n, sort_bins, sort_lb, slices, slice_len, (uint32_t)wb, wpg, row_i0, row_i1, blo, bcnt);
    sortA_colscan_kernel<<<dim3((sort_bins + SORT_THREADS / 64 - 1) / (SORT_THREADS / 64), G), SORT_THREADS, 0, st>>>(histA, bintot, sort_bins, slices);
    sortA_scan_kernel<<<G, SORT_THREADS, 0, st>>>(bintot, binstart, totals, sort_bins, G == 1 ? bases : nullptr, gstart + (size_t)G * P.nb);
    if (G > 1) sort_bases_kernel<<<1, 64, 0, st>>>(totals, bases, gstart + (size_t)G * P.nb, G);
    static const int staged = [] { const char* e = getenv("BBGPU_SORT_STAGED"); return e ? atoi(e) : 3; }();
    if ((staged & 2) && (P.n & 7u) == 0) {
        if (wide) sortA_scatter_staged_kernel<uint16_t><<<dim3(slices, G), SORT_THREADS, 0, st>>>((const uint16_t*)digits, signs, histA, binstart, bases, tmp_entries, P.n, sort_bins, sort_lb, slices,
                                                                                  slice_len, (uint32_t)wb, wpg, idx_stride, P.W, row_i0, row_i1, blo, bcnt);
        else sortA_scatter_staged_kernel<int16_t><<<dim3(slices, G), SORT_THREADS, 0, st>>>((const int16_t*)digits, signs, histA, binstart, bases, tmp_entries, P.n, sort_bins, sort_lb, slices,
                                                                            slice_len, (uint32_t)wb, wpg, idx_stride, P.W, row_i0, row_i1, blo, bcnt);
    } else
    if (wide) sortA_scatter_kernel<uint16_t><<<dim3(slices, G), SORT_THREADS, 0, st>>>((const uint16_t*)digits, signs, histA, binstart, bases, tmp_entries, P.n, sort_bins, sort_lb, slices,
                                                                   slice_len, (uint32_t)wb, wpg, idx_stride, P.W, row_i0, row_i1, blo, bcnt);
    else sortA_scatter_kernel<int16_t><<<dim3(slices, G), SORT_THREADS, 0, st>>>((const int16_t*)digits, signs, histA, binstart, bases, tmp_entries, P.n, sort_bins, sort_lb, slices,
                                                                   slice_len, (uint32_t)wb, wpg, idx_stride, P.W, row_i0, row_i1, blo, bcnt);
    if (!(staged & 1)) sortB_kernel<<<dim3(sort_bins, G), table ? SORT_THREADS : 256, 0, st>>>(tmp_entries, binstart, bases, sorted, gstart, sort_bins, sort_lb, P.nb);
    else if (table) {
        static const int parts_env = [] { const char* e = getenv("BBGPU_SORTB_PARTS"); return e ? std::min((int)SORTB_MAX_PARTS, std::max(1, atoi(e))) : 0; }();
        uint32_t parts = parts_env ? (uint32_t)parts_env : (((uint64_t)n * nw1 >= ((uint64_t)1 << 21) && G <= MSM_MAX_JOBS) ? SORTB_MAX_PARTS : 1u);
        if ((size_t)G * sort_bins * parts * 128 * 4 > LY.histB_bytes) parts = 1;
        if (parts > 1) sortB_count_kernel<SORT_THREADS><<<dim3(sort_bins, G, parts), SORT_THREADS, 0, st>>>(tmp_entries, binstart, bases, histB, sort_bins, parts);
        sortB_staged_kernel<SORT_THREADS><<<dim3(sort_bins, G, parts), SORT_THREADS, 0, st>>>(tmp_entries, binstart, bases, sorted, gstart, sort_bins, sort_lb, P.nb, histB, parts);
    } else sortB_staged_kernel<256><<<dim3(sort_bins, G), 256, 0, st>>>(tmp_entries, binstart, bases, sorted, gstart, sort_bins, sort_lb, P.nb, nullptr, 1u);
    if (tm_acc) HIPCHK(hipEventRecord(ev[2], st));
    const uint32_t total_buckets = G * P.nb;
    const uint64_t m_expected = bshare ? std::max<uint64_t>(1, (uint64_t)n * nw * bcnt / P.nb) : (uint64_t)n * nw;
    const uint32_t merge_buckets = bshare ? bcnt : total_buckets;
    static const int tp_env = [] { const char* e = getenv("BBGPU_THROUGHPUT"); return e ? atoi(e) : -1; }();
    const bool tp = (tp_env < 0 ? hint : tp_env != 0) && jobs == 1;
    constexpr uint32_t TP_MIN_CHUNK = 20;
    uint32_t ch = bshare ? chunk_len_m(m_expected) : chunk_len(n, nw);
    ch = std::max(ch, min_chunk((uint64_t)n * nw));
    if (tp && ch < TP_MIN_CHUNK && !chunk_forced())
        ch = std::max(ch, std::min<uint32_t>(TP_MIN_CHUNK, (uint32_t)(m_expected / (acc_capacity_lanes() / acc_wg_per_cu()))));
    const uint32_t avg_partials = (uint32_t)(m_expected / ((uint64_t)merge_buckets * ch)) + 1;
    uint32_t logG = 0;
    static const uint32_t lanes_log = [] { const char* e = getenv("BBGPU_MERGE_LANES_LOG"); return e ? (uint32_t)std::min(20, std::max(14, atoi(e))) : 16u; }();
    while ((1u << logG) < avg_partials && logG < 6 && ((uint64_t)merge_buckets << (logG + 1)) <= ((uint64_t)1 << lanes_log)) logG++;
    const uint32_t merge_light = std::max(6u, 8u << logG);
    const uint32_t max_chunks = (uint32_t)(((uint64_t)n * nw + ch - 1) / ch);
    static const int fold_env = [] { const char* e = getenv("BBGPU_FOLD_TAIL"); return e ? atoi(e) : 1; }();
    const bool fold = fold_env != 0;
    msm_accumulate_kernel<<<(max_chunks + MSM_THREADS - 1) / MSM_THREADS, MSM_THREADS, acc_lds_reserve(), st>>>(points, sorted, gstart, partials, total_buckets, ch, acc_prio(), fold ? heavy : nullptr);
    if (tm_acc) {
        HIPCHK(hipEventRecord(ev[3], st));
        if (int rc = acc_ring_record(S, st)) return rc;
    } else {
        S.acc_seq = 0;
    }
    if (!fold) HIPCHK(hipMemsetAsync(heavy, 0, HEAVY_IDS * 4, st));
    static const bool quad_tail = [] { const char* e = getenv("BBGPU_QUAD_TAIL"); return !e || atoi(e) != 0; }();
    static const uint64_t quad_merge_max_entries = [] { const char* e = getenv("BBGPU_QUAD_MERGE_MAX_LOG"); return (uint64_t)1 << (e ? std::min(30, std::max(10, atoi(e))) : 21); }();
    static const int quad_merge = [] { const char* e = getenv("BBGPU_QUAD_MERGE"); return e ? atoi(e) : 1; }();
    if (quad_tail && (quad_merge > 1 || (quad_merge == 1 && (uint64_t)n * nw <= quad_merge_max_entries))) {
        uint32_t logQ = 0;
        while ((2u << logQ) < avg_partials && logQ < 4 && ((uint64_t)merge_buckets << (logQ + 3)) <= ((uint64_t)1 << 17)) logQ++;
        if (quad_merge > 1) logQ = std::min(4, quad_merge - 2);
        msm_merge_quad_kernel<<<(uint32_t)((((uint64_t)merge_buckets << (logQ + 2)) + MSM_THREADS - 1) / MSM_THREADS), MSM_THREADS, 0, st>>>(gstart, partials, buckets, heavy, blo, blo + merge_buckets, ch,
                                                                                                                                  std::max(32u, 8u << logQ), logQ);
    } else
    msm_merge_kernel<<<(uint32_t)((((uint64_t)merge_buckets << logG) + MSM_THREADS - 1) / MSM_THREADS), MSM_THREADS, 0, st>>>(gstart, partials, buckets, heavy,
                                                                                                                     blo, blo + merge_buckets, ch, merge_light, logG);
    msm_merge_heavy_kernel<<<HEAVY_WGS, MSM_THREADS, 0, st>>>(gstart, partials, buckets, heavy, ch, heavy + (((size_t)G * P.nb + HEAVY_IDS + 63) & ~(size_t)63));
    if (tm) HIPCHK(hipEventRecord(ev[4], st));

    const uint32_t H = 1u << P.hbits, L = 1u << P.lbits;
    {
        uint32_t* Rr = scratch;
        uint32_t* Cc = scratch + (size_t)G * H * 32;
        uint32_t* const hout = (uint32_t*)ws.h_out + (size_t)PC.hout_group * 64 * 32;
        uint32_t* dest = fold ? hout : texp;
        const uint32_t zero_words = G * 64 * 32;
        static const bool two_step_env = [] { const char* e = getenv("BBGPU_ROWCOL_TWO_STEP"); return !e || atoi(e) != 0; }();
        if (quad_tail && two_step_env && !bshare && rowcol_two_step(P) && (tp || jobs > 1)) {
            uint32_t* segs = (uint32_t*)(p + LY.segs);
            const uint32_t seg_lanes = 2 * (H * L / ROWCOL_SEG);
            msm_rowcol_seg_kernel<<<dim3((seg_lanes + MSM_THREADS - 1) / MSM_THREADS, G), MSM_THREADS, 0, st>>>(buckets, segs, H, L, fold ? dest : nullptr, zero_words);
            msm_segsum_quad_kernel<<<dim3(H + L, G), 64, 0, st>>>(segs, Rr, Cc, H, L);
        } else
        if (quad_tail) msm_rowcol_quad_kernel<<<dim3((bshare ? brow1 - brow0 : H) + L, G), QFOLD_T, 0, st>>>(buckets, Rr, Cc, H, L, fold ? dest : nullptr, zero_words, bshare ? brow0 : 0u,
                                                                                                   bshare ? brow1 - brow0 : H);
        else msm_rowcol_kernel<<<dim3(H + L, G), std::max(H, L), 0, st>>>(buckets, Rr, Cc, H, L, fold ? dest : nullptr, zero_words);
        if (tm) HIPCHK(hipEventRecord(ev[5], st));
        if (!fold) HIPCHK(hipMemsetAsync(texp, 0, (size_t)G * 64 * 128, st));
        if (quad_tail) msm_final_quad_kernel<<<dim3(1 + P.hbits + P.lbits, G), QFOLD_T, 0, st>>>(Rr, Cc, dest, P.hbits, P.lbits);
        else msm_final_kernel<<<dim3(1 + P.hbits + P.lbits, G), std::max(H, L), 0, st>>>(Rr, Cc, dest, P.hbits, P.lbits);
        if (tm) HIPCHK(hipEventRecord(ev[6], st));
    }
    if (!fold) HIPCHK(hipMemcpyAsync((uint32_t*)ws.h_out + (size_t)PC.hout_group * 64 * 32, texp, (size_t)G * 64 * 128, hipMemcpyDeviceToHost, st));
    HIPCHK(hipEventRecord(S.done, st));
    HIPCHK(launch_check());
    S.npieces++;
    S.pending = true;
    return BBGPU_OK;
}

static host::Xyzz group_sum(const MsmSlot& S, const MsmPiece& PC, uint32_t w)
{
    auto pt = [&](uint32_t slot) {
        host::Xyzz q;
        memcpy(&q, (const uint8_t*)S.ws.h_out + ((size_t)(PC.hout_group + w) * 64 + slot) * 128, 128);
        return q;
    };
    host::Xyzz rs = host::g1_infinity();
    for (int k = (int)PC.hbits - 1; k >= 0; --k) rs = host::g1_add(host::g1_dbl(rs), pt(1 + k));
    for (uint32_t k = 0; k < PC.lbits; k++) rs = host::g1_dbl(rs);
    host::Xyzz cs = host::g1_infinity();
    for (int k = (int)PC.lbits - 1; k >= 0; --k) cs = host::g1_add(host::g1_dbl(cs), pt(32 + k));
    return host::g1_add(host::g1_add(rs, cs), pt(0));
}
static int finish_timing(MsmSlot& S, MsmTiming* timing)
{
    if (S.timed && timing) {
        float ms;
        timing->count = 0;
        if (S.timed_light) {
            for (int i = 0; i < 7; i++) timing->ms[timing->count++] = 0.0f;
            HIPCHK(hipEventElapsedTime(&ms, S.ev[2], S.ev[3]));
            timing->ms[3] = ms;
        } else {
            HIPCHK(hipEventElapsedTime(&ms, S.ev[0], S.ev[6]));
            timing->ms[timing->count++] = ms;
            for (int i = 0; i < 6; i++) {
                HIPCHK(hipEventElapsedTime(&ms, S.ev[i], S.ev[i + 1]));
                timing->ms[timing->count++] = ms;
            }
        }
        float exec = timing->ms[3];
        if (S.acc_seq > 1 && g_acc_seq - (S.acc_seq - 1) < (uint64_t)ACC_RING &&
            hipEventElapsedTime(&ms, g_acc_end[(S.acc_seq - 1) % ACC_RING], g_acc_end[S.acc_seq % ACC_RING]) == hipSuccess && ms > 0.0f && ms < exec)
            exec = ms;
        (void)hipGetLastError();
        timing->ms[timing->count++] = exec;
    }
    return BBGPU_OK;
}
int msm_finish(MsmSlot& S, host::Xyzz* result, MsmTiming* timing)
{
    *result = host::g1_infinity();
    if (!S.pending) return BBGPU_ERR_STATE;
    if (S.jobs > 1) return BBGPU_ERR_STATE;
    S.pending = false;
    bool waited = false;
    host::Xyzz total = host::g1_infinity();
    for (int pi = 0; pi < S.npieces; pi++) {
        const MsmPiece& PC = S.piece[pi];
        if (PC.trivial) continue;
        if (!waited) HIPCHK(hipEventSynchronize(S.done));
        waited = true;
        host::Xyzz acc = host::g1_infinity();
        for (int w = (int)PC.nw - 1; w >= 0; --w) {
            for (uint32_t k = 0; k < PC.c; k++) acc = host::g1_dbl(acc);
            acc = host::g1_add(acc, group_sum(S, PC, (uint32_t)w));
        }
        for (uint32_t k = 0; k < PC.c * PC.wb; k++) acc = host::g1_dbl(acc);
        total = host::g1_add(total, acc);
    }
    *result = total;
    if (!waited) return BBGPU_OK;
    return finish_timing(S, timing);
}
int msm_finish_batch(MsmSlot& S, host::Xyzz* results, MsmTiming* timing)
{
    if (S.jobs <= 1) return msm_finish(S, results, timing);
    if (!S.pending) return BBGPU_ERR_STATE;
    S.pending = false;
    for (uint32_t j = 0; j < S.jobs; j++) results[j] = host::g1_infinity();
    bool waited = false;
    for (int pi = 0; pi < S.npieces; pi++) {
        const MsmPiece& PC = S.piece[pi];
        if (PC.trivial) continue;
        if (!waited) HIPCHK(hipEventSynchronize(S.done));
        waited = true;
        for (uint32_t j = 0; j < S.jobs; j++) results[j] = host::g1_add(results[j], group_sum(S, PC, j));
    }
    if (!waited) return BBGPU_OK;
    return finish_timing(S, timing);
}

void MsmSlot::release()
{
    ws.release();
    if (done) (void)hipEventDestroy(done);
    done = nullptr;
    for (auto& e : ev) {
        if (e) (void)hipEventDestroy(e);
        e = nullptr;
    }
    if (stream) (void)hipStreamDestroy(stream);
    stream = nullptr;
    pending = false;
    npieces = 0;
    helper = -1;
    is_helper = append = false;
}

int srs_upload(const uint64_t* host_table, size_t n, uint32_t** d_srs_out, hipStream_t st, size_t stride_bytes)
{
    DevBuf tab, srs;
    HIPCHK(dev_malloc(&tab.p, n * stride_bytes));
    HIPCHK(dev_malloc(&srs.p, n * 64));
    if (int rc = host_to_device(tab.p, host_table, n * stride_bytes, st)) return rc;
    srs_convert_kernel<<<(uint32_t)((n + 127) / 128), 128, 0, st>>>(tab.as<uint32_t>(), srs.as<uint32_t>(), (uint32_t)n, (uint32_t)(stride_bytes / 4));
    HIPCHK(launch_check());
    HIPCHK(hipStreamSynchronize(st));
    *d_srs_out = srs.release<uint32_t>();
    return BBGPU_OK;
}

int srs_upload_into(const uint64_t* host_table, size_t n, uint32_t* d_raw, uint32_t* d_srs, hipStream_t st, size_t stride_bytes)
{
    if (int rc = host_to_device(d_raw, host_table, n * stride_bytes, st)) return rc;
    srs_convert_kernel<<<(uint32_t)((n + 127) / 128), 128, 0, st>>>(d_raw, d_srs, (uint32_t)n, (uint32_t)(stride_bytes / 4));
    HIPCHK(launch_check());
    return BBGPU_OK;
}

int srs_build_table(const uint32_t* d_srs, size_t n, int c, int num_windows, int w_begin, int w_end, uint32_t** d_alloc_out, uint32_t** d_tab_out, hipStream_t st)
{
    DevBuf alloc;
    HIPCHK(dev_malloc(&alloc.p, (size_t)(w_end - w_begin) * n * 64));
    uint32_t* d_tab = alloc.as<uint32_t>() - (size_t)w_begin * n * 16;
    srs_table_kernel<<<(uint32_t)((n + MSM_THREADS - 1) / MSM_THREADS), MSM_THREADS, 0, st>>>(d_srs, d_tab, (uint32_t)n, make_layout(c, true), (uint32_t)num_windows,
                                                                                          (uint32_t)w_begin, (uint32_t)w_end);
    HIPCHK(launch_check());
    HIPCHK(hipStreamSynchronize(st));
    *d_alloc_out = alloc.release<uint32_t>();
    *d_tab_out = d_tab;
    return BBGPU_OK;
}

int srs_generate(const uint64_t* x_mont256, size_t first, size_t n, uint32_t** d_srs_out, uint64_t* host_table_out, hipStream_t st)
{
    DevBuf tab, srs;
    HIPCHK(dev_malloc(&tab.p, 32 * 256 * 128));
    HIPCHK(dev_malloc(&srs.p, n * 64));
    srs_gen_table_kernel<<<1, 32, 0, st>>>(tab.as<uint32_t>());
    uint32_t w[8];
    for (int i = 0; i < 4; i++) { w[2 * i] = (uint32_t)x_mont256[i]; w[2 * i + 1] = (uint32_t)(x_mont256[i] >> 32); }
    Fe<Fr, 1, 2> x261 = m256_to_m261<Fr>(unpack<Fr>(w));
    uint32_t cw[8];
    to_canonical(x261, cw);
    Fe<Fr, 1, 6> xc = unpack<Fr>(cw);
    Limbs9 xl;
    for (int i = 0; i < NL; i++) xl.d[i] = xc.d[i];
    srs_gen_points_kernel<<<(uint32_t)((n + 63) / 64), 64, 0, st>>>(tab.as<uint32_t>(), xl, srs.as<uint32_t>(), (uint32_t)n, (uint32_t)first);
    HIPCHK(launch_check());
    if (host_table_out) {
        DevBuf exp;
        HIPCHK(dev_malloc(&exp.p, n * 128));
        srs_export_kernel<<<(uint32_t)((n + 127) / 128), 128, 0, st>>>(srs.as<uint32_t>(), exp.as<uint32_t>(), (uint32_t)n);
        HIPCHK(launch_check());
        if (int rc = device_to_host_sync(host_table_out, exp.p, n * 128, st)) return rc;
    }
    HIPCHK(hipStreamSynchronize(st));
    *d_srs_out = srs.release<uint32_t>();
    return BBGPU_OK;
}

}
```

Measured before the change: 917.9 million.

## Fuse scalar digit decomposition with sort histogram into one front kernel

```diff
diff --git a/barretenberg_amd/csrc/msm.hip b/barretenberg_amd/csrc/msm.hip
--- a/barretenberg_amd/csrc/msm.hip
+++ b/barretenberg_amd/csrc/msm.hip
@@ -223,67 +223,22 @@
 };
 template <class DT> struct DigitTraits { static constexpr bool wide = false; };
 template <> struct DigitTraits<uint16_t> { static constexpr bool wide = true; };
-template <class DT> __device__ __forceinline__ int load_digit(const DT* __restrict__ dg, const unsigned long long* __restrict__ sg, uint32_t i)
-{
-    if constexpr (DigitTraits<DT>::wide) {
-        const int u = dg[i];
-        return ((sg[i >> 6] >> (i & 63u)) & 1ull) ? -u - 1 : u;
-    } else {
-        return dg[i];
-    }
-}
-template <class DT> __device__ __forceinline__ void load_digits8(const DT* __restrict__ dg, const unsigned long long* __restrict__ sg, uint32_t i8, int (&d)[8])
+template <class DT> __device__ __forceinline__ void load_keys8(const DT* __restrict__ dg, const uint8_t* __restrict__ sb8, uint32_t i8, uint32_t (&key)[8])
 {
     const uint4 q = *reinterpret_cast<const uint4*>(dg + i8);
     const uint32_t w[4] = { q.x, q.y, q.z, q.w };
     if constexpr (DigitTraits<DT>::wide) {
-        const uint32_t sb = reinterpret_cast<const uint8_t*>(sg)[i8 >> 3];
+        const uint32_t sb = sb8[i8 >> 3];
 #pragma unroll
         for (int k = 0; k < 8; k++) {
-            const int u = (int)((w[k >> 1] >> (16 * (k & 1))) & 0xffffu);
-            d[k] = ((sb >> k) & 1u) ? -u - 1 : u;
+            const uint32_t u = (w[k >> 1] >> (16 * (k & 1))) & 0xffffu, neg = (sb >> k) & 1u;
+            key[k] = (u | neg) ? ((u + neg - 1u) | (neg << 31)) : 0xffffffffu;
         }
     } else {
 #pragma unroll
-        for (int k = 0; k < 8; k++) d[k] = (int)(int16_t)(w[k >> 1] >> (16 * (k & 1)));
-    }
-}
-template <class DT> __global__ void __launch_bounds__(MSM_THREADS) msm_digits_kernel(ScalarSets sets, DT* __restrict__ digits_all, unsigned long long* __restrict__ signs_all,
-                                                               uint32_t n, WinLayout LO, uint32_t num_windows, uint32_t wb, uint32_t we)
-{
-    FRONT_PRIO();
-    const uint32_t i = blockIdx.x * blockDim.x + threadIdx.x;
-    if (i >= n) return;
-    const uint32_t* __restrict__ scalars = sets.p[blockIdx.y];
-    DT* __restrict__ digits = digits_all + (size_t)blockIdx.y * num_windows * n;
-    const uint32_t s64 = (n + 63) >> 6;
-    unsigned long long* __restrict__ signs = signs_all + (size_t)blockIdx.y * num_windows * s64;
-    uint32_t w[8], k[9];
-    ld8(scalars + (size_t)i * 8, w);
-    to_canonical(exact_limbs(mul(unpack<Fr>(w), fe_from<Fr>(Fr::M256_TO_PLAIN))), w);
-#pragma unroll
-    for (int j = 0; j < 8; j++) k[j] = w[j];
-    k[8] = 0;
-    uint32_t carry = 0;
-    for (uint32_t win = 0; win < we; win++) {
-        const uint32_t bit = LO.off[win], sz = LO.off[win + 1] - bit, j = bit >> 5, s = bit & 31;
-        const uint32_t half = 1u << (sz - 1), mask = (1u << sz) - 1;
-        uint32_t v = 0;
-        if (j < 8) {
-            v = k[j] >> s;
-            if (s + sz > 32) v |= k[j + 1] << (32 - s);
-        }
-        v = (v & mask) + carry;
-        carry = (win + 1 < num_windows && v >= half) ? 1u : 0u;
-        const int32_t d = (int32_t)v - (int32_t)(carry << sz);
-        if (win >= wb) {
-            if constexpr (DigitTraits<DT>::wide) {
-                const unsigned long long neg = __ballot(d < 0);
-                digits[(size_t)win * n + i] = (DT)(d < 0 ? -d - 1 : d);
-                if ((threadIdx.x & 63u) == 0) signs[(size_t)win * s64 + (i >> 6)] = neg;
-            } else {
-                digits[(size_t)win * n + i] = (DT)d;
-            }
+        for (int k = 0; k < 8; k++) {
+            const int d = (int)(int16_t)(w[k >> 1] >> (16 * (k & 1)));
+            key[k] = d ? (d > 0 ? (uint32_t)(d - 1) : ((uint32_t)(-d - 1) | 0x80000000u)) : 0xffffffffu;
         }
     }
 }
@@ -319,49 +274,82 @@
     if ((todo >> lane) & 1ull) res = atomicAdd(&ctr[key], 1u);
     return res;
 }
-
-template <class DT> __global__ void __launch_bounds__(SORT_THREADS) __attribute__((amdgpu_num_vgpr(32))) sortA_hist_kernel(const DT* __restrict__ digits, const unsigned long long* __restrict__ signs, uint32_t* __restrict__ histA, uint32_t n,
-                                                                uint32_t bins, uint32_t lb, uint32_t slices, uint32_t slice_len, uint32_t win0,
-                                                                uint32_t wpg, uint32_t first_i0, uint32_t last_i1, uint32_t blo, uint32_t bcnt)
+__device__ __forceinline__ void lds_count_dedup(uint32_t* ctr, uint32_t key)
+{
+    bool todo = true;
+    for (int it = 0; it < 4; it++) {
+        const uint64_t act = __ballot(todo);
+        if (!act) return;
+        const int leader = __ffsll((unsigned long long)act) - 1;
+        const uint32_t kk = __builtin_amdgcn_readlane(key, leader);
+        const uint64_t m = __ballot(todo && key == kk);
+        if (__popcll(m) < 2) break;
+        if ((int)__lane_id() == leader) atomicAdd(&ctr[kk], (uint32_t)__popcll(m));
+        todo = todo && key != kk;
+    }
+    if (todo) atomicAdd(&ctr[key], 1u);
+}
+
+constexpr uint32_t FRONT_CTRS = 4096;
+template <class DT> __global__ void __launch_bounds__(SORT_THREADS) msm_front_kernel(ScalarSets sets, DT* __restrict__ digits_all, unsigned long long* __restrict__ signs_all,
+                                                                                    uint32_t* __restrict__ histA, uint32_t n, uint32_t n8, uint32_t base, uint32_t rem,
+                                                                                    uint32_t num_windows, uint32_t wb, uint32_t we, uint32_t bins, uint32_t lb,
+                                                                                    uint32_t slices, uint32_t slice_len, uint32_t table, uint32_t first_i0,
+                                                                                    uint32_t last_i1, uint32_t blo, uint32_t bcnt)
 {
     FRONT_PRIO();
-    __shared__ uint32_t lh[SORT_THREADS];
-    const uint32_t s = blockIdx.x, wl = blockIdx.y;
-    lh[threadIdx.x] = 0;
+    __shared__ uint32_t cnt[FRONT_CTRS];
+    const uint32_t s = blockIdx.x, job = blockIdx.y, t = threadIdx.x;
+    const uint32_t nctr = table ? bins : (we - wb) * bins;
+    for (uint32_t x = t; x < nctr; x += SORT_THREADS) cnt[x] = 0;
     __syncthreads();
-    const uint32_t lo = s * slice_len, hi = min(n, lo + slice_len);
+    const uint32_t* __restrict__ scalars = sets.p[job];
     const uint32_t s64 = (n + 63) >> 6;
-    if ((n & 7u) == 0) {
-        const uint32_t lo8 = lo & ~7u, bpw = lo < hi ? (((hi + 7u) & ~7u) - lo8) >> 3 : 0u;
-        for (uint32_t u = threadIdx.x; u < wpg * bpw; u += SORT_THREADS) {
-            const uint32_t k = u / bpw, i8 = lo8 + (u - k * bpw) * 8;
-            const uint32_t klo = (k == 0) ? max(lo, first_i0) : lo, khi = (k + 1 == wpg) ? min(hi, last_i1) : hi;
-            int d[8];
-            load_digits8<DT>(digits + (size_t)(win0 + wl * wpg + k) * n, signs + (size_t)(win0 + wl * wpg + k) * s64, i8, d);
-            const bool heavy = wave_keys_heavy(d[0] != 0, (uint32_t)((d[0] < 0 ? -d[0] : d[0]) - 1) >> lb);
-#pragma unroll
-            for (int j = 0; j < 8; j++)
-                if (d[j] && i8 + j >= klo && i8 + j < khi) {
-                    const uint32_t b = (uint32_t)((d[j] < 0 ? -d[j] : d[j]) - 1);
-                    if (b - blo < bcnt) (void)lds_inc_dedup(lh, b >> lb, heavy);
-                }
-        }
-    } else {
-        for (uint32_t k = 0; k < wpg; k++) {
-            const DT* dg = digits + (size_t)(win0 + wl * wpg + k) * n;
-            const unsigned long long* sg = signs + (size_t)(win0 + wl * wpg + k) * s64;
-            const uint32_t klo = (k == 0) ? max(lo, first_i0) : lo, khi = (k + 1 == wpg) ? min(hi, last_i1) : hi;
-            for (uint32_t i = klo + threadIdx.x; i < khi; i += SORT_THREADS) {
-                const int d = load_digit<DT>(dg, sg, i);
-                if (d) {
-                    const uint32_t b = (uint32_t)((d < 0 ? -d : d) - 1);
-                    if (b - blo < bcnt) atomicAdd(&lh[b >> lb], 1u);
-                }
+    DT* __restrict__ digits = digits_all + (size_t)job * num_windows * n8;
+    unsigned long long* __restrict__ signs = signs_all + (size_t)job * num_windows * s64;
+    const uint32_t lo = s * slice_len, hi = min(n8, lo + slice_len);
+    for (uint32_t i = lo + t; i < hi; i += SORT_THREADS) {
+        uint32_t k[9];
+#pragma unroll
+        for (int j = 0; j < 9; j++) k[j] = 0;
+        if (i < n) {
+            uint32_t w[8];
+            ld8(scalars + (size_t)i * 8, w);
+            to_canonical(exact_limbs(mul(unpack<Fr>(w), fe_from<Fr>(Fr::M256_TO_PLAIN))), w);
+#pragma unroll
+            for (int j = 0; j < 8; j++) k[j] = w[j];
+        }
+        uint32_t carry = 0, bit = 0;
+        for (uint32_t win = 0; win < we; win++) {
+            const uint32_t sz = base + (win < rem ? 1u : 0u), j = bit >> 5, sh = bit & 31;
+            uint32_t v = 0;
+            if (j < 8) {
+                v = k[j] >> sh;
+                if (sh + sz > 32) v |= k[j + 1] << (32 - sh);
             }
+            bit += sz;
+            v = (v & ((1u << sz) - 1)) + carry;
+            carry = (win + 1 < num_windows && v >= (1u << (sz - 1))) ? 1u : 0u;
+            if (win < wb) continue;
+            int32_t d = (int32_t)v - (int32_t)(carry << sz);
+            const uint32_t b = (uint32_t)((d < 0 ? -d : d) - 1);
+            if (b - blo >= bcnt || (win == wb && i < first_i0) || (win + 1 == we && i >= last_i1)) d = 0;
+            const uint32_t at = win * n8 + i;
+            if constexpr (DigitTraits<DT>::wide) {
+                const unsigned long long neg = __ballot(d < 0);
+                digits[at] = (DT)(d < 0 ? -d - 1 : d);
+                if ((t & 63u) == 0) signs[(size_t)win * s64 + (i >> 6)] = neg;
+            } else {
+                digits[at] = (DT)d;
+            }
+            if (d) lds_count_dedup(cnt, (table ? 0u : (win - wb) * bins) + (b >> lb));
         }
     }
     __syncthreads();
-    if (threadIdx.x < bins) histA[((size_t)wl * slices + s) * bins + threadIdx.x] = lh[threadIdx.x];
+    for (uint32_t x = t; x < nctr; x += SORT_THREADS) {
+        const uint32_t g = table ? job : x / bins, bin = table ? x : x - g * bins;
+        histA[((size_t)g * slices + s) * bins + bin] = cnt[x];
+    }
 }
 
 __global__ void __launch_bounds__(SORT_THREADS) sortA_colscan_kernel(uint32_t* __restrict__ histA, uint32_t* __restrict__ bintot, uint32_t bins,
@@ -433,67 +421,11 @@
 }
 
 
-template <class DT> __global__ void __launch_bounds__(SORT_THREADS) __attribute__((amdgpu_num_vgpr(32))) sortA_scatter_kernel(const DT* __restrict__ digits, const unsigned long long* __restrict__ signs, const uint32_t* __restrict__ cursorsA,
-                                                                   const uint32_t* __restrict__ binstart, const uint32_t* __restrict__ bases,
-                                                                   uint32_t* __restrict__ tmp, uint32_t n, uint32_t bins, uint32_t lb,
-                                                                   uint32_t slices, uint32_t slice_len, uint32_t win0, uint32_t wpg,
-                                                                   uint32_t idx_stride, uint32_t windows_per_job, uint32_t first_i0, uint32_t last_i1, uint32_t blo, uint32_t bcnt)
-{
-    FRONT_PRIO();
-    __shared__ uint32_t lc[SORT_THREADS];
-    const uint32_t s = blockIdx.x, wl = blockIdx.y;
-    if (threadIdx.x < bins)
-        lc[threadIdx.x] = cursorsA[((size_t)wl * slices + s) * bins + threadIdx.x] + binstart[(size_t)wl * bins + threadIdx.x] + bases[wl];
-    __syncthreads();
-    const uint32_t lo = s * slice_len, hi = min(n, lo + slice_len);
-    const uint32_t lomask = (1u << lb) - 1;
-    const uint32_t s64 = (n + 63) >> 6;
-    if ((n & 7u) == 0) {
-        const uint32_t lo8 = lo & ~7u, bpw = lo < hi ? (((hi + 7u) & ~7u) - lo8) >> 3 : 0u;
-        for (uint32_t u = threadIdx.x; u < wpg * bpw; u += SORT_THREADS) {
-            const uint32_t k = u / bpw, i8 = lo8 + (u - k * bpw) * 8;
-            const uint32_t wabs = win0 + wl * wpg + k;
-            const uint32_t row = (wabs % windows_per_job) * idx_stride;
-            const uint32_t klo = (k == 0) ? max(lo, first_i0) : lo, khi = (k + 1 == wpg) ? min(hi, last_i1) : hi;
-            int d[8];
-            load_digits8<DT>(digits + (size_t)wabs * n, signs + (size_t)wabs * s64, i8, d);
-#pragma unroll
-            for (int j = 0; j < 8; j++) {
-                if (d[j] && i8 + j >= klo && i8 + j < khi) {
-                    const uint32_t b = (uint32_t)((d[j] < 0 ? -d[j] : d[j]) - 1);
-                    if (b - blo < bcnt) {
-                        const uint32_t pos = atomicAdd(&lc[b >> lb], 1u);
-                        tmp[pos] = (row + i8 + j) | ((b & lomask) << 24) | (d[j] < 0 ? 0x80000000u : 0u);
-                    }
-                }
-            }
-        }
-        return;
-    }
-    for (uint32_t k = 0; k < wpg; k++) {
-        const uint32_t wabs = win0 + wl * wpg + k;
-        const DT* dg = digits + (size_t)wabs * n;
-        const unsigned long long* sg = signs + (size_t)wabs * s64;
-        const uint32_t row = (wabs % windows_per_job) * idx_stride;
-        const uint32_t klo = (k == 0) ? max(lo, first_i0) : lo, khi = (k + 1 == wpg) ? min(hi, last_i1) : hi;
-        for (uint32_t i = klo + threadIdx.x; i < khi; i += SORT_THREADS) {
-            const int d = load_digit<DT>(dg, sg, i);
-            if (d) {
-                const uint32_t b = (uint32_t)((d < 0 ? -d : d) - 1);
-                if (b - blo < bcnt) {
-                    const uint32_t pos = atomicAdd(&lc[b >> lb], 1u);
-                    tmp[pos] = (row + i) | ((b & lomask) << 24) | (d < 0 ? 0x80000000u : 0u);
-                }
-            }
-        }
-    }
-}
-
-template <class DT> __global__ void __launch_bounds__(SORT_THREADS) __attribute__((amdgpu_waves_per_eu(8, 8))) sortA_scatter_staged_kernel(const DT* __restrict__ digits, const unsigned long long* __restrict__ signs, const uint32_t* __restrict__ cursorsA,
+template <class DT> __global__ void __launch_bounds__(SORT_THREADS) __attribute__((amdgpu_waves_per_eu(8, 8))) sortA_scatter_kernel(const DT* __restrict__ digits, const unsigned long long* __restrict__ signs,
+                                                                          const uint32_t* __restrict__ cursorsA, const uint32_t* __restrict__ bintot,
                                                                           const uint32_t* __restrict__ binstart, const uint32_t* __restrict__ bases,
-                                                                          uint32_t* __restrict__ tmp, uint32_t n, uint32_t bins, uint32_t lb,
-                                                                          uint32_t slices, uint32_t slice_len, uint32_t win0, uint32_t wpg,
-                                                                          uint32_t idx_stride, uint32_t windows_per_job, uint32_t first_i0, uint32_t last_i1, uint32_t blo, uint32_t bcnt)
+                                                                          uint32_t* __restrict__ tmp, uint32_t n, uint32_t n8, uint32_t bins, uint32_t lb,
+                                                                          uint32_t slices, uint32_t slice_len, uint32_t win0, uint32_t wpg, uint32_t idx_stride)
 {
     FRONT_PRIO();
     constexpr uint32_t TILE = SORT_THREADS * 8;
@@ -503,40 +435,53 @@
     __shared__ uint32_t wsum[SORT_THREADS / 64 + 1];
     __shared__ uint32_t buf[TILE];
     __shared__ uint16_t bbin[TILE];
+    __shared__ uint32_t slice_total;
     const uint32_t s = blockIdx.x, wl = blockIdx.y, t = threadIdx.x, lane = t & 63, wave = t >> 6;
-    lc[t] = t < bins ? cursorsA[((size_t)wl * slices + s) * bins + t] + binstart[(size_t)wl * bins + t] + bases[wl] : 0u;
-    const uint32_t lo = s * slice_len, hi = min(n, lo + slice_len);
+    uint32_t mine = 0;
+    if (t < bins) {
+        const size_t h = ((size_t)wl * slices + s) * bins + t;
+        const uint32_t c0 = cursorsA[h];
+        mine = (s + 1 < slices ? cursorsA[h + bins] : bintot[(size_t)wl * bins + t]) - c0;
+        lc[t] = c0 + binstart[(size_t)wl * bins + t] + bases[wl];
+    }
+    if (t == 0) slice_total = 0;
+    __syncthreads();
+    if (mine) atomicAdd(&slice_total, mine);
+    __syncthreads();
+    const bool armed = __syncthreads_or(64 * (uint64_t)mine > slice_total);
     const uint32_t lomask = (1u << lb) - 1;
     const uint32_t s64 = (n + 63) >> 6;
-    const uint32_t lo8 = lo & ~7u, bpw = lo < hi ? (((hi + 7u) & ~7u) - lo8) >> 3 : 0u;
-    const uint32_t total_u = wpg * bpw;
+    const uint32_t lo = s * slice_len, hi = min(n8, lo + slice_len);
+    const uint32_t bpw = lo < hi ? (hi - lo) >> 3 : 0u, total_u = wpg * bpw;
+    const DT* __restrict__ dg = digits + (size_t)(win0 + wl * wpg) * n8;
+    const uint8_t* __restrict__ sg = reinterpret_cast<const uint8_t*>(signs + (size_t)(win0 + wl * wpg) * s64);
+    const uint32_t q = bpw ? SORT_THREADS / bpw : 0u, rr = SORT_THREADS - q * bpw;
+    uint32_t k = bpw ? t / bpw : 0u, r = t - k * bpw;
     for (uint32_t u0 = 0; u0 < total_u; u0 += SORT_THREADS) {
         th[t] = 0;
         __syncthreads();
         uint32_t ent[8], bn[8], rk[8];
-        const uint32_t u = u0 + t;
 #pragma unroll
         for (int j = 0; j < 8; j++) bn[j] = 0xffffffffu;
-        if (u < total_u) {
-            const uint32_t k = u / bpw, i8 = lo8 + (u - k * bpw) * 8;
-            const uint32_t wabs = win0 + wl * wpg + k;
-            const uint32_t row = (wabs % windows_per_job) * idx_stride;
-            const uint32_t klo = (k == 0) ? max(lo, first_i0) : lo, khi = (k + 1 == wpg) ? min(hi, last_i1) : hi;
-            int d[8];
-            load_digits8<DT>(digits + (size_t)wabs * n, signs + (size_t)wabs * s64, i8, d);
-            const bool heavy = wave_keys_heavy(d[0] != 0, (uint32_t)((d[0] < 0 ? -d[0] : d[0]) - 1) >> lb);
+        if (u0 + t < total_u) {
+            const uint32_t i8 = lo + r * 8;
+            const uint32_t idx = (win0 + k) * idx_stride + i8;
+            uint32_t key[8];
+            load_keys8<DT>(dg + k * n8, sg + k * s64 * 8, i8, key);
+            const bool heavy = armed && wave_keys_heavy(key[0] != 0xffffffffu, (key[0] & 0x7fffffffu) >> lb);
 #pragma unroll
             for (int j = 0; j < 8; j++) {
-                if (d[j] && i8 + j >= klo && i8 + j < khi) {
-                    const uint32_t b = (uint32_t)((d[j] < 0 ? -d[j] : d[j]) - 1);
-                    if (b - blo < bcnt) {
-                        bn[j] = b >> lb;
-                        ent[j] = (row + i8 + j) | ((b & lomask) << 24) | (d[j] < 0 ? 0x80000000u : 0u);
-                        rk[j] = lds_inc_dedup(th, bn[j], heavy);
-                    }
+                if (key[j] != 0xffffffffu) {
+                    const uint32_t b = key[j] & 0x7fffffffu;
+                    bn[j] = b >> lb;
+                    ent[j] = (idx + j) | ((b & lomask) << 24) | (key[j] & 0x80000000u);
+                    rk[j] = lds_inc_dedup(th, bn[j], heavy);
                 }
             }
         }
+        r += rr;
+        k += q;
+        if (r >= bpw) { r -= bpw; k++; }
         __syncthreads();
         const uint32_t c = th[t];
         uint32_t incl = c;
@@ -567,63 +512,6 @@
         __syncthreads();
         const uint32_t tile_n = wsum[SORT_THREADS / 64];
         for (uint32_t x = t; x < tile_n; x += SORT_THREADS) tmp[dlt[bbin[x]] + x] = buf[x];
-    }
-}
-
-__global__ void __launch_bounds__(SORT_THREADS) sortB_kernel(const uint32_t* __restrict__ tmp, const uint32_t* __restrict__ binstart,
-                                                   const uint32_t* __restrict__ bases, uint32_t* __restrict__ sorted, uint32_t* __restrict__ gstart,
-                                                   uint32_t bins, uint32_t lb, uint32_t nb)
-{
-    FRONT_PRIO();
-    __shared__ uint32_t cnt[128];
-    __shared__ uint32_t cur[128];
-    const uint32_t bin = blockIdx.x, wl = blockIdx.y, t = threadIdx.x;
-    const uint32_t nlo = 1u << lb;
-    const uint32_t start = bases[wl] + binstart[(size_t)wl * bins + bin];
-    const uint32_t end = (bin + 1 < bins) ? bases[wl] + binstart[(size_t)wl * bins + bin + 1] : bases[wl + 1];
-    if (t < 128) cnt[t] = 0;
-    __syncthreads();
-    constexpr int UB = 8;
-    for (uint32_t e0 = start + t; e0 < end; e0 += UB * blockDim.x) {
-        uint32_t v[UB];
-#pragma unroll
-        for (int k = 0; k < UB; k++) {
-            const uint32_t e = e0 + k * blockDim.x;
-            v[k] = e < end ? tmp[e] : 0u;
-        }
-#pragma unroll
-        for (int k = 0; k < UB; k++)
-            if (e0 + k * blockDim.x < end) atomicAdd(&cnt[(v[k] >> 24) & 0x7f], 1u);
-    }
-    __syncthreads();
-    if (t < 64) {
-        const uint32_t a = cnt[2 * t], b2 = cnt[2 * t + 1], sum = a + b2;
-        uint32_t incl = sum;
-#pragma unroll
-        for (int off = 1; off < 64; off <<= 1) {
-            const uint32_t o = __shfl_up(incl, off);
-            if ((int)t >= off) incl += o;
-        }
-        cur[2 * t] = start + incl - sum;
-        cur[2 * t + 1] = start + incl - sum + a;
-    }
-    __syncthreads();
-    if (t < nlo) gstart[(size_t)wl * nb + (size_t)bin * nlo + t] = cur[t];
-    __syncthreads();
-    for (uint32_t e0 = start + t; e0 < end; e0 += UB * blockDim.x) {
-        uint32_t v[UB];
-#pragma unroll
-        for (int k = 0; k < UB; k++) {
-            const uint32_t e = e0 + k * blockDim.x;
-            v[k] = e < end ? tmp[e] : 0u;
-        }
-#pragma unroll
-        for (int k = 0; k < UB; k++) {
-            if (e0 + k * blockDim.x < end) {
-                const uint32_t pos = atomicAdd(&cur[(v[k] >> 24) & 0x7f], 1u);
-                sorted[pos] = v[k] & 0x80ffffffu;
-            }
-        }
     }
 }
 
@@ -678,6 +566,7 @@
     const uint32_t len = bend - bstart;
     const uint32_t parts = (parts_launched > 1 && len > SORTB_SPLIT_MIN) ? parts_launched : 1u;
     if (part >= parts) return;
+    const bool armed = len > SORTB_SPLIT_MIN || (uint64_t)len * bins > 16 * (uint64_t)(bases[wl + 1] - bases[wl]);
     const uint32_t start = bstart + (uint32_t)(((uint64_t)len * part) / parts), end = bstart + (uint32_t)(((uint64_t)len * (part + 1)) / parts);
     if (t < 128) {
         uint32_t total = 0, before = 0;
@@ -700,7 +589,7 @@
             const uint32_t e = e0 + k * THREADS;
             v[k] = e < end ? tmp[e] : 0u;
         }
-        const bool heavy = wave_keys_heavy(e0 < end, (v[0] >> 24) & 0x7f);
+        const bool heavy = armed && wave_keys_heavy(e0 < end, (v[0] >> 24) & 0x7f);
 #pragma unroll
         for (int k = 0; k < UB; k++)
             if (e0 + k * THREADS < end) (void)lds_inc_dedup(cnt, (v[k] >> 24) & 0x7f, heavy);
@@ -731,7 +620,7 @@
             const uint32_t e = base + k * THREADS + t;
             v[k] = e < end ? tmp[e] : 0u;
         }
-        const bool heavy = wave_keys_heavy(base + t < end, (v[0] >> 24) & 0x7f);
+        const bool heavy = armed && wave_keys_heavy(base + t < end, (v[0] >> 24) & 0x7f);
 #pragma unroll
         for (int k = 0; k < UB; k++) {
             rk[k] = 0u;
@@ -1360,7 +1249,7 @@
 }
 
 struct MsmPlan {
-    uint32_t n, c, W, nb, hbits, lbits, slices, slice_len, sort_lb, sort_bins;
+    uint32_t n, c, W, nb, hbits, lbits, slices, hist_slices, slice_len, sort_lb, sort_bins;
 };
 constexpr uint32_t ACC_LDS_RESERVE = 41 * 1024;
 static uint32_t acc_wg_per_cu()
@@ -1467,6 +1356,7 @@
     P.sort_bins = P.nb >> P.sort_lb;
     if ((uint64_t)P.slices * 4096 > n) P.slices = std::max<uint32_t>(1, (uint32_t)(n / 4096));
     P.slice_len = (uint32_t)((n + P.slices - 1) / P.slices);
+    P.hist_slices = std::max<uint32_t>(P.slices, (uint32_t)std::min<size_t>(256, n / 1024));
     return P;
 }
 
@@ -1480,9 +1370,9 @@
     MsmCarve L;
     size_t p = 0;
     const size_t wmax = std::max<size_t>(P.W, nw);
-    L.digits = p;      p += al(wmax * n * 2);
+    L.digits = p;      p += al(wmax * ((n + 7) & ~(size_t)7) * 2);
     L.signs = p;       p += al(wmax * ((n + 63) / 64) * 8);
-    L.histA = p;       p += al(nw * P.slices * 1024 * 4);
+    L.histA = p;       p += al(nw * P.hist_slices * 1024 * 4);
     L.histB_bytes = (uint64_t)n * nw >= ((uint64_t)1 << 21) ? (size_t)MSM_MAX_JOBS * 1024 * SORTB_MAX_PARTS * 128 * 4 : 0;
     L.histB = p;       p += al(L.histB_bytes);
     L.binstart = p;    p += al(nw * 1024 * 4 + 256);
@@ -1617,12 +1507,14 @@
     }
     uint32_t slices = table ? std::max<uint32_t>(1, P.slices * nw1 / 2) : P.slices;
     if (table && jobs == 1) {
-        const uint32_t by_cap = (uint32_t)(((uint64_t)nw * P.slices * 1024) / ((uint64_t)G * sort_bins));
+        const uint32_t by_cap = (uint32_t)(((uint64_t)nw * P.hist_slices * 1024) / ((uint64_t)G * sort_bins));
         const uint32_t want = std::min<uint32_t>(std::min<uint32_t>(208, (uint32_t)(n / 2048)), by_cap);
         slices = std::max(slices, want);
     }
+    if (!table) slices = P.hist_slices;
     if (const char* e = getenv("BBGPU_SLICES")) slices = std::min<uint32_t>(std::max(1, atoi(e)), P.slices * nw1);
-    const uint32_t slice_len = (uint32_t)((n + slices - 1) / slices);
+    const uint32_t n8 = (uint32_t)((n + 7) & ~(size_t)7);
+    const uint32_t slice_len = (uint32_t)((((n + slices - 1) / slices) + 63) & ~(size_t)63);
     const uint32_t idx_stride = table ? (uint32_t)tab_stride : 0u;
     const uint32_t* points = table ? d_tab : d_srs;
     PC.c = P.c; PC.nw = G; PC.wb = table ? 0u : (uint32_t)wb; PC.hbits = P.hbits; PC.lbits = P.lbits;
@@ -1657,7 +1549,7 @@
     uint32_t* buckets = (uint32_t*)(p + LY.buckets);
     uint32_t* scratch = (uint32_t*)(p + LY.arena);
     uint32_t* texp = (uint32_t*)(p + LY.texp);
-    if ((uint64_t)G * slices * sort_bins > (uint64_t)nw * P.slices * 1024 || sort_bins > 1024 ||
+    if ((uint64_t)G * slices * sort_bins > (uint64_t)nw * P.hist_slices * 1024 || sort_bins > 1024 || (table ? sort_bins : nw1 * sort_bins) > FRONT_CTRS ||
         (size_t)G * ((size_t)(1u << P.hbits) + (size_t)(1u << P.lbits)) + 64 > arena_points(P, G)) {
         set_error("internal: MSM launch shape exceeds the workspace layout");
         return BBGPU_ERR_STATE;
@@ -1684,27 +1576,20 @@
     ScalarSets sets{};
     for (int j = 0; j < jobs; j++) sets.p[j] = (const uint32_t*)d_scalars_v[j];
     const bool wide = c > 16;
-    if (wide) msm_digits_kernel<uint16_t><<<dim3((P.n + MSM_THREADS - 1) / MSM_THREADS, jobs), MSM_THREADS, 0, st>>>(sets, (uint16_t*)digits, signs, P.n, make_layout(c, table), P.W, (uint32_t)wb, (uint32_t)we);
-    else msm_digits_kernel<int16_t><<<dim3((P.n + MSM_THREADS - 1) / MSM_THREADS, jobs), MSM_THREADS, 0, st>>>(sets, (int16_t*)digits, signs, P.n, make_layout(c, table), P.W, (uint32_t)wb, (uint32_t)we);
+    const uint32_t lay_base = table ? SCALAR_BITS / P.W : P.c, lay_rem = table ? SCALAR_BITS - lay_base * P.W : 0u;
+    if (wide) msm_front_kernel<uint16_t><<<dim3(slices, jobs), SORT_THREADS, 0, st>>>(sets, (uint16_t*)digits, signs, histA, P.n, n8, lay_base, lay_rem, P.W, (uint32_t)wb, (uint32_t)we,
+                                                                                   sort_bins, sort_lb, slices, slice_len, table, row_i0, row_i1, blo, bcnt);
+    else msm_front_kernel<int16_t><<<dim3(slices, jobs), SORT_THREADS, 0, st>>>(sets, (int16_t*)digits, signs, histA, P.n, n8, lay_base, lay_rem, P.W, (uint32_t)wb, (uint32_t)we,
+                                                                             sort_bins, sort_lb, slices, slice_len, table, row_i0, row_i1, blo, bcnt);
     if (tm) HIPCHK(hipEventRecord(ev[1], st));
-    if (wide) sortA_hist_kernel<uint16_t><<<dim3(slices, G), SORT_THREADS, 0, st>>>((const uint16_t*)digits, signs, histA, P.n, sort_bins, sort_lb, slices, slice_len, (uint32_t)wb, wpg, row_i0, row_i1, blo, bcnt);
-    else sortA_hist_kernel<int16_t><<<dim3(slices, G), SORT_THREADS, 0, st>>>((const int16_t*)digits, signs, histA, P.n, sort_bins, sort_lb, slices, slice_len, (uint32_t)wb, wpg, row_i0, row_i1, blo, bcnt);
     sortA_colscan_kernel<<<dim3((sort_bins + SORT_THREADS / 64 - 1) / (SORT_THREADS / 64), G), SORT_THREADS, 0, st>>>(histA, bintot, sort_bins, slices);
     sortA_scan_kernel<<<G, SORT_THREADS, 0, st>>>(bintot, binstart, totals, sort_bins, G == 1 ? bases : nullptr, gstart + (size_t)G * P.nb);
     if (G > 1) sort_bases_kernel<<<1, 64, 0, st>>>(totals, bases, gstart + (size_t)G * P.nb, G);
-    static const int staged = [] { const char* e = getenv("BBGPU_SORT_STAGED"); return e ? atoi(e) : 3; }();
-    if ((staged & 2) && (P.n & 7u) == 0) {
-        if (wide) sortA_scatter_staged_kernel<uint16_t><<<dim3(slices, G), SORT_THREADS, 0, st>>>((const uint16_t*)digits, signs, histA, binstart, bases, tmp_entries, P.n, sort_bins, sort_lb, slices,
-                                                                                  slice_len, (uint32_t)wb, wpg, idx_stride, P.W, row_i0, row_i1, blo, bcnt);
-        else sortA_scatter_staged_kernel<int16_t><<<dim3(slices, G), SORT_THREADS, 0, st>>>((const int16_t*)digits, signs, histA, binstart, bases, tmp_entries, P.n, sort_bins, sort_lb, slices,
-                                                                            slice_len, (uint32_t)wb, wpg, idx_stride, P.W, row_i0, row_i1, blo, bcnt);
-    } else
-    if (wide) sortA_scatter_kernel<uint16_t><<<dim3(slices, G), SORT_THREADS, 0, st>>>((const uint16_t*)digits, signs, histA, binstart, bases, tmp_entries, P.n, sort_bins, sort_lb, slices,
-                                                                   slice_len, (uint32_t)wb, wpg, idx_stride, P.W, row_i0, row_i1, blo, bcnt);
-    else sortA_scatter_kernel<int16_t><<<dim3(slices, G), SORT_THREADS, 0, st>>>((const int16_t*)digits, signs, histA, binstart, bases, tmp_entries, P.n, sort_bins, sort_lb, slices,
-                                                                   slice_len, (uint32_t)wb, wpg, idx_stride, P.W, row_i0, row_i1, blo, bcnt);
-    if (!(staged & 1)) sortB_kernel<<<dim3(sort_bins, G), table ? SORT_THREADS : 256, 0, st>>>(tmp_entries, binstart, bases, sorted, gstart, sort_bins, sort_lb, P.nb);
-    else if (table) {
+    if (wide) sortA_scatter_kernel<uint16_t><<<dim3(slices, G), SORT_THREADS, 0, st>>>((const uint16_t*)digits, signs, histA, bintot, binstart, bases, tmp_entries, P.n, n8, sort_bins, sort_lb,
+                                                                                  slices, slice_len, (uint32_t)wb, wpg, idx_stride);
+    else sortA_scatter_kernel<int16_t><<<dim3(slices, G), SORT_THREADS, 0, st>>>((const int16_t*)digits, signs, histA, bintot, binstart, bases, tmp_entries, P.n, n8, sort_bins, sort_lb,
+                                                                            slices, slice_len, (uint32_t)wb, wpg, idx_stride);
+    if (table) {
         static const int parts_env = [] { const char* e = getenv("BBGPU_SORTB_PARTS"); return e ? std::min((int)SORTB_MAX_PARTS, std::max(1, atoi(e))) : 0; }();
         uint32_t parts = parts_env ? (uint32_t)parts_env : (((uint64_t)n * nw1 >= ((uint64_t)1 << 21) && G <= MSM_MAX_JOBS) ? SORTB_MAX_PARTS : 1u);
         if ((size_t)G * sort_bins * parts * 128 * 4 > LY.histB_bytes) parts = 1;
```

After: 919.9 million, median of 6. About the same (+0.2%).
